# microsoft/BLAS-on-flash

Measured on NVIDIA B200. Metric: gemm_gflops, higher is better.
Workload: dtype f32

## Files before the change

### blas-on-flash_b200/csrc/common.cuh

```cuda
#pragma once

#include <cuda.h>
#include <cuda_runtime.h>

#include <atomic>
#include <cstdarg>
#include <cstdint>
#include <cstdio>
#include <cstring>
#include <mutex>
#include <string>
#include <vector>

#include "bof_b200.h"

namespace bof {

constexpr int kNumSmsFallback = 148;

struct StageSlot {
  void* ptr = nullptr;
  cudaEvent_t ev = nullptr;
  bool in_flight = false;
  char* out_dst = nullptr;
  size_t out_pitch = 0, out_width = 0, out_rows = 0;
};

class CopyPool;
class Drainer;

}

namespace bof { struct CommState; }

struct bof_ctx {
  bof_config cfg{};
  int device = 0;
  int num_sms = bof::kNumSmsFallback;
  size_t l2_bytes = 0;
  cudaStream_t compute = nullptr;
  cudaStream_t h2d = nullptr;
  cudaStream_t d2h = nullptr;
  std::vector<bof::StageSlot> stage_in, stage_out;
  bof::CopyPool* pool = nullptr;
  bof::CopyPool* pool_out = nullptr;
  bof::Drainer* drainer = nullptr;
  std::string err;
  bof_stats stats{};
  std::atomic<int64_t> launches{0};
  void* tmap_encode = nullptr;
  static constexpr int kSlots = 40;
  void* slot_ptr[kSlots] = {};
  size_t slot_bytes[kSlots] = {};
  std::vector<cudaEvent_t> events;
  struct TraceMark { cudaEvent_t ev; const char* what; int idx; };
  std::vector<TraceMark> trace;
  std::vector<cudaEvent_t> trace_pool;
  struct HostMark { double ms; const char* what; long idx; };
  std::vector<HostMark> host_trace;
  std::mutex host_trace_mu;
  double trace_t0 = 0.0;
  cudaEvent_t tk0 = nullptr, tk1 = nullptr;
  bool tk_valid = false;
  uint32_t* sync_ctr = nullptr;
  size_t sync_ctr_count = 0;
  bof::CommState* comm = nullptr;
  cudaStream_t coll = nullptr;
  int sm_reserve = 0;
};

namespace bof {

struct PerDeviceOnce {
  std::atomic<uint64_t> mask{0};
  bool need(int dev) const { return ((mask.load(std::memory_order_acquire) >> (dev & 63)) & 1ull) == 0; }
  void done(int dev) { mask.fetch_or(1ull << (dev & 63), std::memory_order_release); }
};

inline int fail(bof_ctx* ctx, int code, const char* fmt, ...) {
  char buf[512];
  va_list ap;
  va_start(ap, fmt);
  vsnprintf(buf, sizeof(buf), fmt, ap);
  va_end(ap);
  if (ctx) ctx->err = buf;
  if (getenv("BOF_VERBOSE")) fprintf(stderr, "[bof_b200] error %d: %s\n", code, buf);
  return code;
}

#define BOF_CUDA(ctx, expr)                                                                  \
  do {                                                                                       \
    cudaError_t e__ = (expr);                                                                \
    if (e__ != cudaSuccess)                                                                  \
      return bof::fail((ctx), BOF_ECUDA, "%s failed: %s (%s:%d)", #expr,                     \
                       cudaGetErrorString(e__), __FILE__, __LINE__);                         \
  } while (0)

#define BOF_LAUNCH_CHECK(ctx, what)                                                          \
  do {                                                                                       \
    cudaError_t e__ = cudaGetLastError();                                                    \
    if (e__ != cudaSuccess)                                                                  \
      return bof::fail((ctx), BOF_ECUDA, "launch of %s failed: %s (%s:%d)", (what),          \
                       cudaGetErrorString(e__), __FILE__, __LINE__);                         \
    (ctx)->launches.fetch_add(1, std::memory_order_relaxed);                                 \
  } while (0)

#define BOF_REQUIRE(ctx, cond, ...)                                                          \
  do {                                                                                       \
    if (!(cond)) return bof::fail((ctx), BOF_EINVAL, __VA_ARGS__);                           \
  } while (0)

template <typename T>
__host__ __device__ constexpr T ceil_div(T a, T b) {
  return (a + b - 1) / b;
}
template <typename T>
__host__ __device__ constexpr T round_up(T a, T b) {
  return ceil_div(a, b) * b;
}

inline bool aligned16(const void* p) { return (reinterpret_cast<uintptr_t>(p) & 15) == 0; }

int slot_reserve(bof_ctx* ctx, int slot, size_t bytes, void** out);
template <typename T>
int slot_reserve(bof_ctx* ctx, int slot, size_t count, T** out) {
  void* p = nullptr;
  int rc = slot_reserve(ctx, slot, count * sizeof(T), &p);
  *out = static_cast<T*>(p);
  return rc;
}


int launch_spmm_rm(bof_ctx* ctx, cudaStream_t s, int64_t m, int64_t k, float alpha,
                   const float* vals, const int32_t* idx, const int64_t* offs, const float* B,
                   int64_t ldb, float beta, float* C, int64_t ldc, int64_t b_rows = 0);
int launch_spmv(bof_ctx* ctx, cudaStream_t s, char trans, int64_t m, int64_t n, const float* vals,
                const int32_t* idx, const int64_t* offs, const float* x, float* y, int64_t nnz = -1);
size_t spmv_t_workspace_bytes(int64_t n, int64_t nnz);
int launch_spmv_t_sorted(bof_ctx* ctx, cudaStream_t s, int accumulate, int64_t m, int64_t n, int64_t nnz, const float* vals,
                         const int32_t* idx, const int64_t* offs, const float* x, float* y, void* ws, size_t ws_bytes);
constexpr int kSlotSpmvT = 35;
constexpr int kSlotSpmmLong = 36;
int launch_idx_narrow(bof_ctx* ctx, cudaStream_t s, const int64_t* in, int32_t* out, int64_t n);
int launch_idx_widen(bof_ctx* ctx, cudaStream_t s, const int32_t* in, int64_t* out, int64_t n);
int launch_transpose(bof_ctx* ctx, cudaStream_t s, int64_t rows, int64_t cols, const float* in,
                     int64_t ldi, float* out, int64_t ldo);
int launch_add_outer_terms(bof_ctx* ctx, cudaStream_t s, float* C, int64_t rows, int64_t cols, int64_t ldc,
                           const float* rowv, const float* colv, int row_first);
int launch_transpose_axpby(bof_ctx* ctx, cudaStream_t s, int64_t rows, int64_t cols, float alpha,
                           const float* in, int64_t ldi, float beta, float* out, int64_t ldo);

int launch_split_planes(bof_ctx* ctx, cudaStream_t s, int64_t R, int64_t K, const float* src,
                        int64_t s_r, int64_t s_k, float* hi, float* lo, int64_t kp);

struct GemmEpilogue {
  float alpha = 1.f, beta = 0.f;
  float* C = nullptr;
  int64_t ldc = 0;
  const float* row_add = nullptr;
  const float* col_add = nullptr;
  int32_t* argmin_out = nullptr;
  const float* carry = nullptr;
  int64_t ld_carry = 0;
  bool raw_out = false;
};

int launch_gemm_tc(bof_ctx* ctx, cudaStream_t s, int cta_group, int64_t M, int64_t N, int64_t K,
                   int64_t kp, const float* p_hi, const float* p_lo, const float* q_hi,
                   const float* q_lo, const GemmEpilogue& ep, int64_t k_chunk);

int tc_issue_rate(bof_ctx* ctx, cudaStream_t s, int kind, int rounds, double* mma_tflops, double* useful_tflops);

int launch_gemm_ffma(bof_ctx* ctx, cudaStream_t s, int64_t M, int64_t N, int64_t K, float alpha,
                     const float* A, int64_t a_r, int64_t a_k, const float* B, int64_t b_k,
                     int64_t b_c, float beta, float* C, int64_t ldc);

int launch_row_sqnorm(bof_ctx* ctx, cudaStream_t s, int64_t rows, int64_t dim, const float* X,
                      int64_t ldx, float* out);
size_t kmeans_reduce_workspace_bytes(int64_t npoints, int64_t ncenters, int64_t dim);
int launch_kmeans_reduce_ws(bof_ctx* ctx, cudaStream_t s, int64_t npoints, int64_t ncenters,
                            int64_t dim, const float* points, const int32_t* assign, float* sums,
                            float* counts, void* ws, size_t ws_bytes, float* counts_hi = nullptr);
int launch_kmeans_finalize(bof_ctx* ctx, cudaStream_t s, int64_t ncenters, int64_t dim,
                           const float* sums, const float* counts, float* centers, float* c_l2sq,
                           const float* counts_hi = nullptr);

size_t csr2csc_workspace_bytes(int64_t m, int64_t n, int64_t nnz);
int launch_csr2csc(bof_ctx* ctx, cudaStream_t s, int64_t m, int64_t n, int64_t nnz,
                   const int64_t* offs, const int32_t* idx, const float* vals, int64_t* offs_t,
                   int32_t* idx_t, float* vals_t, void* ws, size_t ws_bytes);

}
```

### blas-on-flash_b200/csrc/gemm_tc.cu

```cuda
#include "common.cuh"

#include <cuda_bf16.h>

#ifndef BOF_DEFAULT_HYBRID
#define BOF_DEFAULT_HYBRID 1
#endif

namespace bof {
namespace tc {

constexpr int BLOCK_M = 128;
constexpr int BLOCK_K = 32;
constexpr int UMMA_K = 8;
constexpr int LOAD_N = 128;
constexpr int STAGES = 3;
constexpr int PLANE_BYTES = 128 * BLOCK_K * 4;
constexpr int STAGE_BYTES = 4 * PLANE_BYTES;
constexpr int NUM_THREADS = 384;
constexpr int NUM_EPI_WARPS = 8;
constexpr uint32_t PEER_BIT_MASK = 0xFEFFFFFFu;

enum EpiMode { EPI_GEMM = 0, EPI_ARGMIN = 1 };

struct Params {
  int64_t M, N;
  int32_t num_kb;
  int32_t kb_per_chunk;
  int32_t tiles_m, tiles_n;
  int32_t n_per_item;
  float alpha, beta;
  float* C;
  int64_t ldc;
  const float* row_add;
  const float* col_add;
  int32_t* argmin_out;
  uint32_t* sync_counters;
  int32_t sync_kb;
  const float* carry;
  int64_t ld_carry;
  int32_t raw_out;
};

__device__ __forceinline__ uint32_t smem_u32(const void* p) {
  return static_cast<uint32_t>(__cvta_generic_to_shared(p));
}
__device__ __forceinline__ uint32_t cluster_ctarank() {
  uint32_t r;
  asm volatile("mov.u32 %0, %%cluster_ctarank;" : "=r"(r));
  return r;
}
__device__ __forceinline__ void cluster_sync_all() {
  asm volatile("barrier.cluster.arrive.release.aligned;\n\tbarrier.cluster.wait.acquire.aligned;" ::: "memory");
}
__device__ __forceinline__ void mbar_init(uint64_t* bar, uint32_t count) {
  asm volatile("mbarrier.init.shared::cta.b64 [%0], %1;" ::"r"(smem_u32(bar)), "r"(count));
}
__device__ __forceinline__ void fence_barrier_init() {
  asm volatile("fence.mbarrier_init.release.cluster;" ::: "memory");
}
__device__ __forceinline__ uint64_t globaltimer_ns() {
  uint64_t t;
  asm volatile("mov.u64 %0, %%globaltimer;" : "=l"(t));
  return t;
}
__device__ __forceinline__ void mbar_wait(uint64_t* bar, uint32_t parity) {
  const uint32_t addr = smem_u32(bar);
  uint32_t done = 0;
  uint64_t t0 = 0;
  uint32_t spins = 0;
  while (true) {
    asm volatile(
        "{\n\t.reg .pred p;\n\t"
        "mbarrier.try_wait.parity.shared::cta.b64 p, [%1], %2;\n\t"
        "selp.u32 %0, 1, 0, p;\n\t}"
        : "=r"(done)
        : "r"(addr), "r"(parity)
        : "memory");
    if (done) break;
    if ((++spins & 0xfffu) == 0) {
      const uint64_t now = globaltimer_ns();
      if (t0 == 0) t0 = now;
      else if (now - t0 > 4000000000ull) __trap();
    }
  }
}
__device__ __forceinline__ void mbar_arrive_expect_tx(uint64_t* bar, uint32_t bytes) {
  asm volatile("mbarrier.arrive.expect_tx.shared::cta.b64 _, [%0], %1;" ::"r"(smem_u32(bar)), "r"(bytes)
               : "memory");
}
__device__ __forceinline__ void mbar_arrive_leader(uint64_t* bar) {
  asm volatile("mbarrier.arrive.shared::cluster.b64 _, [%0];" ::"r"(smem_u32(bar) & PEER_BIT_MASK) : "memory");
}

template <int CG>
__device__ __forceinline__ void tma_load_2d(const CUtensorMap* map, uint64_t* full_bar, void* dst,
                                            int32_t c_inner, int32_t c_outer) {
  if constexpr (CG == 2) {
    asm volatile(
        "cp.async.bulk.tensor.2d.cta_group::2.shared::cluster.global.mbarrier::complete_tx::bytes"
        " [%0], [%1, {%3, %4}], [%2];" ::"r"(smem_u32(dst)),
        "l"(reinterpret_cast<uint64_t>(map)), "r"(smem_u32(full_bar) & PEER_BIT_MASK), "r"(c_inner),
        "r"(c_outer)
        : "memory");
  } else {
    asm volatile(
        "cp.async.bulk.tensor.2d.shared::cluster.global.mbarrier::complete_tx::bytes"
        " [%0], [%1, {%3, %4}], [%2];" ::"r"(smem_u32(dst)),
        "l"(reinterpret_cast<uint64_t>(map)), "r"(smem_u32(full_bar)), "r"(c_inner), "r"(c_outer)
        : "memory");
  }
}

template <int CG>
__device__ __forceinline__ void tmem_alloc(uint32_t* dst_smem, uint32_t ncols) {
  if constexpr (CG == 2) {
    asm volatile("tcgen05.alloc.cta_group::2.sync.aligned.shared::cta.b32 [%0], %1;" ::"r"(smem_u32(dst_smem)), "r"(ncols) : "memory");
    asm volatile("tcgen05.relinquish_alloc_permit.cta_group::2.sync.aligned;" ::: "memory");
  } else {
    asm volatile("tcgen05.alloc.cta_group::1.sync.aligned.shared::cta.b32 [%0], %1;" ::"r"(smem_u32(dst_smem)), "r"(ncols) : "memory");
    asm volatile("tcgen05.relinquish_alloc_permit.cta_group::1.sync.aligned;" ::: "memory");
  }
}
template <int CG>
__device__ __forceinline__ void tmem_dealloc(uint32_t taddr, uint32_t ncols) {
  if constexpr (CG == 2)
    asm volatile("tcgen05.dealloc.cta_group::2.sync.aligned.b32 %0, %1;" ::"r"(taddr), "r"(ncols) : "memory");
  else
    asm volatile("tcgen05.dealloc.cta_group::1.sync.aligned.b32 %0, %1;" ::"r"(taddr), "r"(ncols) : "memory");
}
__device__ __forceinline__ void tc_fence_before() {
  asm volatile("tcgen05.fence::before_thread_sync;" ::: "memory");
}
__device__ __forceinline__ void tc_fence_after() {
  asm volatile("tcgen05.fence::after_thread_sync;" ::: "memory");
}

template <int CG>
__device__ __forceinline__ void umma_tf32(uint32_t tmem_d, uint64_t desc_a, uint64_t desc_b,
                                          uint32_t idesc, uint32_t accumulate) {
  if constexpr (CG == 2) {
    asm volatile(
        "{\n\t.reg .pred p;\n\tsetp.ne.b32 p, %4, 0;\n\t"
        "tcgen05.mma.cta_group::2.kind::tf32 [%0], %1, %2, %3, p;\n\t}" ::"r"(tmem_d),
        "l"(desc_a), "l"(desc_b), "r"(idesc), "r"(accumulate)
        : "memory");
  } else {
    asm volatile(
        "{\n\t.reg .pred p;\n\tsetp.ne.b32 p, %4, 0;\n\t"
        "tcgen05.mma.cta_group::1.kind::tf32 [%0], %1, %2, %3, p;\n\t}" ::"r"(tmem_d),
        "l"(desc_a), "l"(desc_b), "r"(idesc), "r"(accumulate)
        : "memory");
  }
}
template <int CG>
__device__ __forceinline__ void umma_bf16(uint32_t tmem_d, uint64_t desc_a, uint64_t desc_b,
                                          uint32_t idesc, uint32_t accumulate) {
  if constexpr (CG == 2) {
    asm volatile(
        "{\n\t.reg .pred p;\n\tsetp.ne.b32 p, %4, 0;\n\t"
        "tcgen05.mma.cta_group::2.kind::f16 [%0], %1, %2, %3, p;\n\t}" ::"r"(tmem_d),
        "l"(desc_a), "l"(desc_b), "r"(idesc), "r"(accumulate)
        : "memory");
  } else {
    asm volatile(
        "{\n\t.reg .pred p;\n\tsetp.ne.b32 p, %4, 0;\n\t"
        "tcgen05.mma.cta_group::1.kind::f16 [%0], %1, %2, %3, p;\n\t}" ::"r"(tmem_d),
        "l"(desc_a), "l"(desc_b), "r"(idesc), "r"(accumulate)
        : "memory");
  }
}
template <int CG>
__device__ __forceinline__ void umma_commit(uint64_t* bar) {
  if constexpr (CG == 2) {
    const uint16_t mask = 0b11;
    asm volatile(
        "tcgen05.commit.cta_group::2.mbarrier::arrive::one.shared::cluster.multicast::cluster.b64 [%0], %1;" ::"r"(
            smem_u32(bar)),
        "h"(mask)
        : "memory");
  } else {
    asm volatile("tcgen05.commit.cta_group::1.mbarrier::arrive::one.shared::cluster.b64 [%0];" ::"r"(smem_u32(bar))
                 : "memory");
  }
}
__device__ __forceinline__ void tmem_ld32(uint32_t taddr, uint32_t (&v)[32]) {
  asm volatile(
      "tcgen05.ld.sync.aligned.32x32b.x32.b32 "
      "{%0, %1, %2, %3, %4, %5, %6, %7, %8, %9, %10, %11, %12, %13, %14, %15, "
      "%16, %17, %18, %19, %20, %21, %22, %23, %24, %25, %26, %27, %28, %29, %30, %31}, [%32];"
      : "=r"(v[0]), "=r"(v[1]), "=r"(v[2]), "=r"(v[3]), "=r"(v[4]), "=r"(v[5]), "=r"(v[6]),
        "=r"(v[7]), "=r"(v[8]), "=r"(v[9]), "=r"(v[10]), "=r"(v[11]), "=r"(v[12]), "=r"(v[13]),
        "=r"(v[14]), "=r"(v[15]), "=r"(v[16]), "=r"(v[17]), "=r"(v[18]), "=r"(v[19]), "=r"(v[20]),
        "=r"(v[21]), "=r"(v[22]), "=r"(v[23]), "=r"(v[24]), "=r"(v[25]), "=r"(v[26]), "=r"(v[27]),
        "=r"(v[28]), "=r"(v[29]), "=r"(v[30]), "=r"(v[31])
      : "r"(taddr)
      : "memory");
}
__device__ __forceinline__ void tmem_ld_wait() {
  asm volatile("tcgen05.wait::ld.sync.aligned;" ::: "memory");
}

__device__ __forceinline__ uint64_t make_smem_desc(uint32_t saddr) {
  uint64_t d = 0;
  d |= (uint64_t)((saddr >> 4) & 0x3FFF);
  d |= (uint64_t)1 << 16;
  d |= (uint64_t)(1024 >> 4) << 32;
  d |= (uint64_t)1 << 46;
  d |= (uint64_t)2 << 61;
  return d;
}
__host__ __device__ constexpr uint32_t make_idesc(int umma_m, int umma_n, uint32_t fmt = 2u) {
  return (1u << 4)
         | (fmt << 7) | (fmt << 10)
         | ((uint32_t)(umma_n >> 3) << 17) | ((uint32_t)(umma_m >> 4) << 24);
}

template <int N>
__device__ __forceinline__ void setmaxnreg_inc() {
  asm volatile("setmaxnreg.inc.sync.aligned.u32 %0;" ::"n"(N));
}
template <int N>
__device__ __forceinline__ void setmaxnreg_dec() {
  asm volatile("setmaxnreg.dec.sync.aligned.u32 %0;" ::"n"(N));
}

struct SmemTail {
  uint64_t full[STAGES];
  uint64_t empty[STAGES];
  uint64_t tmem_full[2];
  uint64_t tmem_empty[2];
  uint32_t tmem_base;
  uint32_t pad;
  float red_val[BLOCK_M];
  int32_t red_idx[BLOCK_M];
};

constexpr size_t SMEM_BYTES = (size_t)STAGES * STAGE_BYTES + sizeof(SmemTail) + 1024;

template <int CG, int EPI, bool CHUNKED, bool HYB, bool FOLD = false>
__global__ void __launch_bounds__(NUM_THREADS, 1)
gemm3xtf32_kernel(const __grid_constant__ CUtensorMap map_p_hi, const __grid_constant__ CUtensorMap map_p_lo,
                  const __grid_constant__ CUtensorMap map_q_hi, const __grid_constant__ CUtensorMap map_q_lo,
                  const Params prm) {
  constexpr int BLOCK_N = (CG == 2) ? 256 : 128;
  constexpr int TILE_M = BLOCK_M * CG;
  constexpr int EPI_COLS = BLOCK_N / 2;
  constexpr uint32_t TMEM_COLS = 2 * BLOCK_N;
  constexpr uint32_t IDESC = make_idesc(BLOCK_M * CG, BLOCK_N, 2u);
  constexpr uint32_t IDESC_BF16 = make_idesc(BLOCK_M * CG, BLOCK_N, 1u);
  static_assert(!FOLD || (EPI == EPI_GEMM && CHUNKED), "the fold carry exists for the chunked GEMM epilogue only");

  extern __shared__ uint8_t smem_raw[];
  uint8_t* smem = reinterpret_cast<uint8_t*>((reinterpret_cast<uintptr_t>(smem_raw) + 1023) & ~(uintptr_t)1023);
  SmemTail* tail = reinterpret_cast<SmemTail*>(smem + (size_t)STAGES * STAGE_BYTES);

  const int warp = threadIdx.x >> 5;
  const int lane = threadIdx.x & 31;
  const uint32_t cta_rank = (CG == 2) ? cluster_ctarank() : 0u;
  const bool is_leader = cta_rank == 0;
  const int cluster_id = blockIdx.x / CG;
  const int num_clusters = gridDim.x / CG;

  if (warp == 1 && lane == 0) {
    for (int s = 0; s < STAGES; ++s) {
      mbar_init(&tail->full[s], CG);
      mbar_init(&tail->empty[s], 1);
    }
    for (int b = 0; b < 2; ++b) {
      mbar_init(&tail->tmem_full[b], 1);
      mbar_init(&tail->tmem_empty[b], NUM_EPI_WARPS * CG);
    }
    fence_barrier_init();
  }
  if (warp == 2) tmem_alloc<CG>(&tail->tmem_base, TMEM_COLS);
  tc_fence_before();
  if constexpr (CG == 2) cluster_sync_all(); else __syncthreads();
  tc_fence_after();
  const uint32_t tmem_base = tail->tmem_base;

  const int num_items = (EPI == EPI_ARGMIN) ? prm.tiles_m : prm.tiles_m * prm.tiles_n;
  const int num_chunks = (prm.num_kb + prm.kb_per_chunk - 1) / prm.kb_per_chunk;

  auto decode_item = [&](int item, int& tm, int& tn0) {
    if (EPI == EPI_ARGMIN) { tm = item; tn0 = 0; return; }
    constexpr int GROUP = 8;
    const int per_group = GROUP * prm.tiles_n;
    const int g = item / per_group;
    const int first_m = g * GROUP;
    const int gsz = min(GROUP, prm.tiles_m - first_m);
    const int r = item - g * per_group;
    tm = first_m + r % gsz;
    tn0 = r / gsz;
  };

  if (warp < 4) {
    if constexpr (CHUNKED) setmaxnreg_dec<40>();
    if (warp == 0) {
      int stage = 0;
      uint32_t phase = 0;
      for (int item = cluster_id; item < num_items; item += num_clusters) {
        int tm, tn0;
        decode_item(item, tm, tn0);
        const int32_t row_p = tm * TILE_M + (int)cta_rank * BLOCK_M;
        for (int nt = 0; nt < prm.n_per_item; ++nt) {
          const int32_t row_q = (tn0 + nt) * BLOCK_N + (int)cta_rank * LOAD_N;
          for (int kb = 0; kb < prm.num_kb; ++kb) {
            mbar_wait(&tail->empty[stage], phase ^ 1);
            if (EPI == EPI_GEMM && prm.sync_kb > 0 && is_leader && lane == 0 && kb % prm.sync_kb == 0) {
              const int wave = (item - cluster_id) / num_clusters;
              const int syncs_per_tile = (prm.num_kb + prm.sync_kb - 1) / prm.sync_kb;
              const uint32_t expected = (uint32_t)min(num_clusters, num_items - wave * num_clusters);
              uint32_t* ctr = prm.sync_counters + (size_t)wave * syncs_per_tile + kb / prm.sync_kb;
              asm volatile("red.release.gpu.global.add.u32 [%0], 1;" ::"l"(ctr) : "memory");
              uint32_t seen = 0;
              const uint64_t t0 = globaltimer_ns();
              for (uint32_t spins = 0;; ++spins) {
                asm volatile("ld.acquire.gpu.global.u32 %0, [%1];" : "=r"(seen) : "l"(ctr) : "memory");
                if (seen >= expected) break;
                __nanosleep(100);
                if ((spins & 0x3fu) == 0x3fu && globaltimer_ns() - t0 > 500000ull) break;
              }
            }
            if (lane == 0) {
              uint8_t* st = smem + (size_t)stage * STAGE_BYTES;
              if (is_leader) mbar_arrive_expect_tx(&tail->full[stage], STAGE_BYTES * CG);
              else mbar_arrive_leader(&tail->full[stage]);
              const int32_t kc = kb * BLOCK_K;
              tma_load_2d<CG>(&map_p_hi, &tail->full[stage], st, kc, row_p);
              tma_load_2d<CG>(&map_p_lo, &tail->full[stage], st + PLANE_BYTES, kc, row_p);
              tma_load_2d<CG>(&map_q_hi, &tail->full[stage], st + 2 * PLANE_BYTES, kc, row_q);
              tma_load_2d<CG>(&map_q_lo, &tail->full[stage], st + 3 * PLANE_BYTES, kc, row_q);
            }
            __syncwarp();
            if (++stage == STAGES) { stage = 0; phase ^= 1; }
          }
        }
      }
    } else if (warp == 1 && is_leader) {
      int stage = 0;
      uint32_t phase = 0;
      uint32_t acc_iter = 0;
      for (int item = cluster_id; item < num_items; item += num_clusters) {
        for (int nt = 0; nt < prm.n_per_item; ++nt) {
          for (int c = 0; c < num_chunks; ++c, ++acc_iter) {
            const uint32_t buf = acc_iter & 1u;
            mbar_wait(&tail->tmem_empty[buf], ((acc_iter >> 1) & 1u) ^ 1u);
            tc_fence_after();
            const uint32_t tmem_d = tmem_base + buf * BLOCK_N;
            const int kb_end = min(prm.num_kb, (c + 1) * prm.kb_per_chunk);
            for (int kb = c * prm.kb_per_chunk; kb < kb_end; ++kb) {
              mbar_wait(&tail->full[stage], phase);
              tc_fence_after();
              if (lane == 0) {
                const uint32_t st = smem_u32(smem + (size_t)stage * STAGE_BYTES);
                const uint64_t d_p_hi = make_smem_desc(st);
                const uint64_t d_p_lo = make_smem_desc(st + PLANE_BYTES);
                const uint64_t d_q_hi = make_smem_desc(st + 2 * PLANE_BYTES);
                const uint64_t d_q_lo = make_smem_desc(st + 3 * PLANE_BYTES);
                const uint32_t fresh = (kb == c * prm.kb_per_chunk) ? 0u : 1u;
                if constexpr (HYB) {
#pragma unroll
                  for (int kk = 0; kk < 2; ++kk) {
                    const uint64_t adv = (uint64_t)(kk * 2);
                    umma_bf16<CG>(tmem_d, d_p_lo + 4 + adv, d_q_lo + adv, IDESC_BF16, kk == 0 ? fresh : 1u);
                    umma_bf16<CG>(tmem_d, d_p_lo + adv, d_q_lo + 4 + adv, IDESC_BF16, 1u);
                  }
#pragma unroll
                  for (int kk = 0; kk < BLOCK_K / UMMA_K; ++kk) {
                    const uint64_t adv = (uint64_t)((kk * UMMA_K * 4) >> 4);
                    umma_tf32<CG>(tmem_d, d_p_hi + adv, d_q_hi + adv, IDESC, 1u);
                  }
                } else {
#pragma unroll
                  for (int kk = 0; kk < BLOCK_K / UMMA_K; ++kk) {
                    const uint64_t adv = (uint64_t)((kk * UMMA_K * 4) >> 4);
                    umma_tf32<CG>(tmem_d, d_p_lo + adv, d_q_hi + adv, IDESC, kk == 0 ? fresh : 1u);
                    umma_tf32<CG>(tmem_d, d_p_hi + adv, d_q_lo + adv, IDESC, 1u);
                    umma_tf32<CG>(tmem_d, d_p_hi + adv, d_q_hi + adv, IDESC, 1u);
                  }
                }
                umma_commit<CG>(&tail->empty[stage]);
                if (kb == kb_end - 1) umma_commit<CG>(&tail->tmem_full[buf]);
              }
              __syncwarp();
              if (++stage == STAGES) { stage = 0; phase ^= 1; }
            }
          }
        }
      }
    }
  } else {
    if constexpr (CHUNKED) setmaxnreg_inc<232>();
    const int e = warp - 4;
    const int quarter = e & 3;
    const int half = e >> 2;
    const int row_in_tile = (int)cta_rank * BLOCK_M + quarter * 32 + lane;
    const uint32_t lane_addr = (uint32_t)(quarter * 32) << 16;
    uint32_t acc_iter = 0;

    for (int item = cluster_id; item < num_items; item += num_clusters) {
      int tm, tn0;
      decode_item(item, tm, tn0);
      const int64_t row = (int64_t)tm * TILE_M + row_in_tile;
      float best = 3.402823466e+38f;
      int32_t best_idx = 0x7fffffff;
      float radd = 0.f;
      if (EPI == EPI_ARGMIN && row < prm.M) radd = __ldg(prm.row_add + row);

      for (int nt = 0; nt < prm.n_per_item; ++nt) {
        const int64_t col0 = (int64_t)(tn0 + nt) * BLOCK_N + half * EPI_COLS;
        float acc[CHUNKED ? EPI_COLS : 1];
        for (int c = 0; c < num_chunks; ++c, ++acc_iter) {
          const uint32_t buf = acc_iter & 1u;
          mbar_wait(&tail->tmem_full[buf], (acc_iter >> 1) & 1u);
          tc_fence_after();
          const uint32_t taddr = tmem_base + lane_addr + buf * BLOCK_N + half * EPI_COLS;
#pragma unroll
          for (int g = 0; g < EPI_COLS / 32; ++g) {
            uint32_t v[32];
            tmem_ld32(taddr + g * 32, v);
            tmem_ld_wait();
            if constexpr (CHUNKED) {
              if (FOLD && c == 0 && prm.carry != nullptr && row < prm.M) {
                const float* krow = prm.carry + row * prm.ld_carry + col0 + g * 32;
#pragma unroll
                for (int j = 0; j < 32; ++j)
                  acc[g * 32 + j] = (col0 + g * 32 + j < prm.N) ? krow[j] + __uint_as_float(v[j]) : __uint_as_float(v[j]);
              } else if (c == 0) {
#pragma unroll
                for (int j = 0; j < 32; ++j) acc[g * 32 + j] = __uint_as_float(v[j]);
              } else {
#pragma unroll
                for (int j = 0; j < 32; ++j) acc[g * 32 + j] += __uint_as_float(v[j]);
              }
            } else {
              if constexpr (EPI == EPI_GEMM) {
                if (row < prm.M) {
                  float* crow = prm.C + row * prm.ldc + col0 + g * 32;
#pragma unroll
                  for (int j = 0; j < 32; ++j) {
                    if (col0 + g * 32 + j < prm.N) {
                      float r = prm.alpha * __uint_as_float(v[j]);
                      if (prm.beta != 0.f) r = fmaf(prm.beta, crow[j], r);
                      crow[j] = r;
                    }
                  }
                }
              } else {
#pragma unroll
                for (int j = 0; j < 32; ++j) {
                  const int64_t cj = col0 + g * 32 + j;
                  if (cj < prm.N) {
                    float d = __fadd_rn(__fadd_rn(-2.f * __uint_as_float(v[j]), __ldg(prm.col_add + cj)), radd);
                    d = fabsf(d);
                    if (d < best) { best = d; best_idx = (int32_t)cj; }
                  }
                }
              }
            }
          }
          tc_fence_before();
          __syncwarp();
          if (lane == 0) mbar_arrive_leader(&tail->tmem_empty[buf]);
        }
        if constexpr (CHUNKED) {
          if constexpr (EPI == EPI_GEMM) {
            if (row < prm.M) {
              float* crow = prm.C + row * prm.ldc + col0;
#pragma unroll
              for (int j = 0; j < EPI_COLS; ++j) {
                if (FOLD && prm.raw_out) {
                  if (col0 + j < prm.N) crow[j] = acc[j];
                } else if (col0 + j < prm.N) {
                  float r = prm.alpha * acc[j];
                  if (prm.beta != 0.f) r = fmaf(prm.beta, crow[j], r);
                  crow[j] = r;
                }
              }
            }
          } else {
#pragma unroll
            for (int j = 0; j < EPI_COLS; ++j) {
              const int64_t cj = col0 + j;
              if (cj < prm.N) {
                float d = __fadd_rn(__fadd_rn(-2.f * acc[j], __ldg(prm.col_add + cj)), radd);
                d = fabsf(d);
                if (d < best) { best = d; best_idx = (int32_t)cj; }
              }
            }
          }
        }
      }

      if constexpr (EPI == EPI_ARGMIN) {
        const int r_local = quarter * 32 + lane;
        if (half == 1) {
          tail->red_val[r_local] = best;
          tail->red_idx[r_local] = best_idx;
        }
        asm volatile("bar.sync 1, 256;" ::: "memory");
        if (half == 0) {
          const float ov = tail->red_val[r_local];
          const int32_t oi = tail->red_idx[r_local];
          if (ov < best || (ov == best && oi < best_idx)) { best = ov; best_idx = oi; }
          if ((uint32_t)best_idx >= (uint32_t)prm.N) best_idx = 0;
          if (row < prm.M) prm.argmin_out[row] = best_idx;
        }
        asm volatile("bar.sync 1, 256;" ::: "memory");
      }
    }
  }

  tc_fence_before();
  if constexpr (CG == 2) cluster_sync_all(); else __syncthreads();
  if (warp == 2) tmem_dealloc<CG>(tmem_base, TMEM_COLS);
}


__global__ void __launch_bounds__(128, 1)
tc_issue_rate_kernel(int kind, int rounds) {
  constexpr int CG = 2;
  constexpr int BLOCK_N = 256;
  constexpr uint32_t IDESC = make_idesc(BLOCK_M * CG, BLOCK_N, 2u);
  constexpr uint32_t IDESC_BF16 = make_idesc(BLOCK_M * CG, BLOCK_N, 1u);
  extern __shared__ uint8_t smem_raw[];
  uint8_t* smem = reinterpret_cast<uint8_t*>((reinterpret_cast<uintptr_t>(smem_raw) + 1023) & ~(uintptr_t)1023);
  __shared__ uint64_t done_bar;
  __shared__ uint32_t tmem_base_s;
  const int warp = threadIdx.x >> 5, lane = threadIdx.x & 31;
  const bool is_leader = cluster_ctarank() == 0;
  uint32_t* w = reinterpret_cast<uint32_t*>(smem);
  for (int i = threadIdx.x; i < STAGE_BYTES / 4; i += blockDim.x) w[i] = 0x3f800000u + ((i * 2654435761u) & 0x007f0000u);
  if (threadIdx.x == 0) { mbar_init(&done_bar, 1); fence_barrier_init(); }
  if (warp == 2) tmem_alloc<CG>(&tmem_base_s, 2 * BLOCK_N);
  asm volatile("fence.proxy.async.shared::cta;" ::: "memory");
  tc_fence_before();
  cluster_sync_all();
  tc_fence_after();
  const uint32_t tmem_d = tmem_base_s;
  if (warp == 1 && is_leader) {
    if (lane == 0) {
      const uint32_t st = smem_u32(smem);
      const uint64_t d_p_hi = make_smem_desc(st), d_p_lo = make_smem_desc(st + PLANE_BYTES);
      const uint64_t d_q_hi = make_smem_desc(st + 2 * PLANE_BYTES), d_q_lo = make_smem_desc(st + 3 * PLANE_BYTES);
      for (int r = 0; r < rounds; ++r) {
        if (kind != 0) {
#pragma unroll
          for (int kk = 0; kk < 2; ++kk) {
            const uint64_t adv = (uint64_t)(kk * 2);
            umma_bf16<CG>(tmem_d, d_p_lo + 4 + adv, d_q_lo + adv, IDESC_BF16, (r | kk) == 0 ? 0u : 1u);
            umma_bf16<CG>(tmem_d, d_p_lo + adv, d_q_lo + 4 + adv, IDESC_BF16, 1u);
          }
        }
        if (kind != 1) {
#pragma unroll
          for (int kk = 0; kk < BLOCK_K / UMMA_K; ++kk) {
            const uint64_t adv = (uint64_t)((kk * UMMA_K * 4) >> 4);
            umma_tf32<CG>(tmem_d, d_p_hi + adv, d_q_hi + adv, IDESC, (kind == 0 && (r | kk) == 0) ? 0u : 1u);
          }
        }
      }
      umma_commit<CG>(&done_bar);
    }
    __syncwarp();
  }
  if (warp == 0) mbar_wait(&done_bar, 0);
  tc_fence_before();
  cluster_sync_all();
  if (warp == 2) tmem_dealloc<CG>(tmem_d, 2 * BLOCK_N);
}

}

namespace {

__device__ __forceinline__ float rna_tf32(float x) {
  uint32_t u;
  asm("cvt.rna.tf32.f32 %0, %1;" : "=r"(u) : "f"(x));
  return __uint_as_float(u);
}

struct SplitElem {
  float hi, lo;
  uint16_t bh, bl;
};
__device__ __forceinline__ SplitElem split_elem(float x) {
  SplitElem s;
  const uint32_t ax = __float_as_uint(x) & 0x7fffffffu;
  if (ax >= 0x7f800000u) {
    s.hi = x; s.lo = 0.f; s.bh = 0; s.bl = 0;
    return s;
  }
  s.hi = ax >= 0x7f7ff000u ? __uint_as_float(__float_as_uint(x) & ~0x1fffu) : rna_tf32(x);
  const float e = x - s.hi;
  s.lo = rna_tf32(e);
  const uint32_t ah = __float_as_uint(s.hi) & 0x7fffffffu;
  s.bh = ah >= 0x7f7f8000u ? (uint16_t)(__float_as_uint(s.hi) >> 16) : __bfloat16_as_ushort(__float2bfloat16_rn(s.hi));
  s.bl = __bfloat16_as_ushort(__float2bfloat16_rn(e));
  return s;
}
__device__ __forceinline__ uint8_t* combo_ptr(float* plane, int64_t r, int64_t kp, int64_t kk, bool lo_half) {
  return reinterpret_cast<uint8_t*>(plane + r * kp) + (kk >> 5) * 128 + (lo_half ? 64 : 0) + (kk & 31) * 2;
}

__global__ void __launch_bounds__(256)
split_planes_kmajor_kernel(int64_t R, int64_t K, const float* __restrict__ src, int64_t s_r,
                           float* __restrict__ hi, float* __restrict__ lo, int64_t kp, bool vec, bool combo) {
  const int64_t quads_per_row = kp / 4;
  const int64_t total = R * quads_per_row;
  const int64_t stride = (int64_t)gridDim.x * blockDim.x;
  for (int64_t q = (int64_t)blockIdx.x * blockDim.x + threadIdx.x; q < total; q += stride) {
    const int64_t r = q / quads_per_row, k0 = (q - r * quads_per_row) * 4;
    float x[4] = {0.f, 0.f, 0.f, 0.f};
    const float* p = src + r * s_r + k0;
    if (vec && k0 + 4 <= K) {
      const float4 t = __ldcs(reinterpret_cast<const float4*>(p));
      x[0] = t.x; x[1] = t.y; x[2] = t.z; x[3] = t.w;
    } else {
#pragma unroll
      for (int u = 0; u < 4; ++u)
        if (k0 + u < K) x[u] = p[u];
    }
    const SplitElem s0 = split_elem(x[0]), s1 = split_elem(x[1]), s2 = split_elem(x[2]), s3 = split_elem(x[3]);
    *reinterpret_cast<float4*>(hi + r * kp + k0) = make_float4(s0.hi, s1.hi, s2.hi, s3.hi);
    if (!combo) {
      *reinterpret_cast<float4*>(lo + r * kp + k0) = make_float4(s0.lo, s1.lo, s2.lo, s3.lo);
    } else {
      uint2 ph, pl;
      ph.x = s0.bh | ((uint32_t)s1.bh << 16);
      ph.y = s2.bh | ((uint32_t)s3.bh << 16);
      pl.x = s0.bl | ((uint32_t)s1.bl << 16);
      pl.y = s2.bl | ((uint32_t)s3.bl << 16);
      *reinterpret_cast<uint2*>(combo_ptr(lo, r, kp, k0, false)) = ph;
      *reinterpret_cast<uint2*>(combo_ptr(lo, r, kp, k0, true)) = pl;
    }
  }
}

__global__ void __launch_bounds__(256)
split_planes_transpose_kernel(int64_t R, int64_t K, const float* __restrict__ src, int64_t s_k,
                              float* __restrict__ hi, float* __restrict__ lo, int64_t kp,
                              unsigned tiles_k, bool combo) {
  __shared__ float tile[32][33];
  const int tx = threadIdx.x & 31, ty = threadIdx.x >> 5;
  const int64_t r0 = (int64_t)(blockIdx.x / tiles_k) * 32, k0 = (int64_t)(blockIdx.x % tiles_k) * 32;
#pragma unroll
  for (int i = ty; i < 32; i += 8) {
    const int64_t kk = k0 + i, r = r0 + tx;
    tile[i][tx] = (kk < K && r < R) ? src[kk * s_k + r] : 0.f;
  }
  __syncthreads();
#pragma unroll
  for (int i = ty; i < 32; i += 8) {
    const int64_t r = r0 + i, kk = k0 + tx;
    if (r < R && kk < kp) {
      const SplitElem sp = split_elem(tile[tx][i]);
      hi[r * kp + kk] = sp.hi;
      if (!combo) {
        lo[r * kp + kk] = sp.lo;
      } else {
        *reinterpret_cast<uint16_t*>(combo_ptr(lo, r, kp, kk, false)) = sp.bh;
        *reinterpret_cast<uint16_t*>(combo_ptr(lo, r, kp, kk, true)) = sp.bl;
      }
    }
  }
}

__global__ void __launch_bounds__(256)
gemm_ffma_kernel(int64_t M, int64_t N, int64_t K, float alpha, const float* __restrict__ A,
                 int64_t a_r, int64_t a_k, const float* __restrict__ B, int64_t b_k, int64_t b_c,
                 float beta, float* __restrict__ C, int64_t ldc) {
  constexpr int BM = 64, BN = 64, BK = 16;
  __shared__ float As[BK][BM + 4];
  __shared__ float Bs[BK][BN + 4];
  const int tid = threadIdx.x;
  const int tx = tid & 15, ty = tid >> 4;
  const int64_t m0 = (int64_t)blockIdx.y * BM, n0 = (int64_t)blockIdx.x * BN;
  float acc[4][4] = {};
  for (int64_t k0 = 0; k0 < K; k0 += BK) {
    for (int i = tid; i < BM * BK; i += 256) {
      int mm, kk;
      if (a_k == 1) { kk = i % BK; mm = i / BK; } else { mm = i % BM; kk = i / BM; }
      const int64_t gm = m0 + mm, gk = k0 + kk;
      As[kk][mm] = (gm < M && gk < K) ? A[gm * a_r + gk * a_k] : 0.f;
    }
    for (int i = tid; i < BN * BK; i += 256) {
      int nn, kk;
      if (b_k == 1) { kk = i % BK; nn = i / BK; } else { nn = i % BN; kk = i / BN; }
      const int64_t gn = n0 + nn, gk = k0 + kk;
      Bs[kk][nn] = (gn < N && gk < K) ? B[gk * b_k + gn * b_c] : 0.f;
    }
    __syncthreads();
#pragma unroll
    for (int kk = 0; kk < BK; ++kk) {
      float a[4], b[4];
#pragma unroll
      for (int u = 0; u < 4; ++u) { a[u] = As[kk][ty * 4 + u]; b[u] = Bs[kk][tx * 4 + u]; }
#pragma unroll
      for (int u = 0; u < 4; ++u)
#pragma unroll
        for (int v = 0; v < 4; ++v) acc[u][v] = fmaf(a[u], b[v], acc[u][v]);
    }
    __syncthreads();
  }
#pragma unroll
  for (int u = 0; u < 4; ++u) {
    const int64_t gm = m0 + ty * 4 + u;
    if (gm >= M) continue;
#pragma unroll
    for (int v = 0; v < 4; ++v) {
      const int64_t gn = n0 + tx * 4 + v;
      if (gn >= N) continue;
      float r = alpha * acc[u][v];
      if (beta != 0.f) r = fmaf(beta, C[gm * ldc + gn], r);
      C[gm * ldc + gn] = r;
    }
  }
}

bool hybrid_split(const bof_ctx* ctx) { return ctx->cfg.gemm_split == 2 || (ctx->cfg.gemm_split == 0 && BOF_DEFAULT_HYBRID); }

typedef CUresult (*EncodeTiledFn)(CUtensorMap*, CUtensorMapDataType, cuuint32_t, void*, const cuuint64_t*,
                                  const cuuint64_t*, const cuuint32_t*, const cuuint32_t*,
                                  CUtensorMapInterleave, CUtensorMapSwizzle, CUtensorMapL2promotion,
                                  CUtensorMapFloatOOBfill);

int make_plane_map(bof_ctx* ctx, CUtensorMap* map, const float* plane, int64_t rows, int64_t kp) {
  BOF_REQUIRE(ctx, ctx->tmap_encode != nullptr, "cuTensorMapEncodeTiled unavailable");
  const cuuint64_t dims[2] = {(cuuint64_t)kp, (cuuint64_t)rows};
  const cuuint64_t strides[1] = {(cuuint64_t)kp * sizeof(float)};
  const cuuint32_t box[2] = {(cuuint32_t)tc::BLOCK_K, 128u};
  const cuuint32_t estr[2] = {1u, 1u};
  CUresult r = reinterpret_cast<EncodeTiledFn>(ctx->tmap_encode)(
      map, CU_TENSOR_MAP_DATA_TYPE_FLOAT32, 2, const_cast<float*>(plane), dims, strides, box, estr,
      CU_TENSOR_MAP_INTERLEAVE_NONE, CU_TENSOR_MAP_SWIZZLE_128B, CU_TENSOR_MAP_L2_PROMOTION_L2_256B,
      CU_TENSOR_MAP_FLOAT_OOB_FILL_NONE);
  if (r != CUDA_SUCCESS) return fail(ctx, BOF_ECUDA, "cuTensorMapEncodeTiled failed with CUresult %d", (int)r);
  return BOF_OK;
}

template <int CG, int EPI, bool CHUNKED, bool HYB, bool FOLD = false>
int launch_variant(bof_ctx* ctx, cudaStream_t s, const CUtensorMap* maps, const tc::Params& prm, int num_items) {
  auto kern = tc::gemm3xtf32_kernel<CG, EPI, CHUNKED, HYB, FOLD>;
  static PerDeviceOnce attr_set;
  if (attr_set.need(ctx->device)) {
    BOF_CUDA(ctx, cudaFuncSetAttribute(kern, cudaFuncAttributeMaxDynamicSharedMemorySize, (int)tc::SMEM_BYTES));
    attr_set.done(ctx->device);
  }
  const int max_clusters = std::max(1, (ctx->num_sms - ctx->sm_reserve) / CG);
  const int clusters = std::max(1, std::min(num_items, max_clusters));
  cudaLaunchConfig_t cfg{};
  cfg.gridDim = dim3((unsigned)(clusters * CG));
  cfg.blockDim = dim3(tc::NUM_THREADS);
  cfg.dynamicSmemBytes = tc::SMEM_BYTES;
  cfg.stream = s;
  cudaLaunchAttribute attr[1];
  attr[0].id = cudaLaunchAttributeClusterDimension;
  attr[0].val.clusterDim.x = CG;
  attr[0].val.clusterDim.y = 1;
  attr[0].val.clusterDim.z = 1;
  cfg.attrs = attr;
  cfg.numAttrs = 1;
  if (!ctx->tk0) {
    BOF_CUDA(ctx, cudaEventCreate(&ctx->tk0));
    BOF_CUDA(ctx, cudaEventCreate(&ctx->tk1));
  }
  BOF_CUDA(ctx, cudaEventRecord(ctx->tk0, s));
  BOF_CUDA(ctx, cudaLaunchKernelEx(&cfg, kern, maps[0], maps[1], maps[2], maps[3], prm));
  BOF_LAUNCH_CHECK(ctx, "gemm3xtf32_kernel");
  BOF_CUDA(ctx, cudaEventRecord(ctx->tk1, s));
  ctx->tk_valid = true;
  return BOF_OK;
}

}

int launch_split_planes(bof_ctx* ctx, cudaStream_t s, int64_t R, int64_t K, const float* src,
                        int64_t s_r, int64_t s_k, float* hi, float* lo, int64_t kp) {
  BOF_REQUIRE(ctx, kp % 32 == 0 && kp >= K, "split: bad padded k");
  if (R == 0) return BOF_OK;
  if (s_k == 1) {
    const bool vec = (s_r % 4 == 0) && aligned16(src);
    const int64_t total = R * (kp / 4);
    const unsigned grid = (unsigned)std::min<int64_t>(ceil_div<int64_t>(total, 256), (int64_t)ctx->num_sms * 32);
    split_planes_kmajor_kernel<<<grid, 256, 0, s>>>(R, K, src, s_r, hi, lo, kp, vec, hybrid_split(ctx));
    BOF_LAUNCH_CHECK(ctx, "split_planes_kmajor_kernel");
  } else {
    BOF_REQUIRE(ctx, s_r == 1, "split: one of the operand strides must be 1");
    const int64_t tiles_k = kp / 32, tiles_r = ceil_div<int64_t>(R, 32);
    BOF_REQUIRE(ctx, tiles_k * tiles_r < (1ll << 31), "split: operand too large for one launch");
    split_planes_transpose_kernel<<<(unsigned)(tiles_k * tiles_r), 256, 0, s>>>(R, K, src, s_k, hi, lo, kp,
                                                                               (unsigned)tiles_k, hybrid_split(ctx));
    BOF_LAUNCH_CHECK(ctx, "split_planes_transpose_kernel");
  }
  return BOF_OK;
}

int launch_gemm_tc(bof_ctx* ctx, cudaStream_t s, int cta_group, int64_t M, int64_t N, int64_t K,
                   int64_t kp, const float* p_hi, const float* p_lo, const float* q_hi,
                   const float* q_lo, const GemmEpilogue& ep, int64_t k_chunk) {
  (void)K;
  if (M == 0 || N == 0) return BOF_OK;
  BOF_REQUIRE(ctx, cta_group == 1 || cta_group == 2, "gemm_tc: cta_group must be 1 or 2");
  BOF_REQUIRE(ctx, kp % 32 == 0 && kp > 0, "gemm_tc: padded k must be a positive multiple of 32");
  BOF_REQUIRE(ctx, M < (1ll << 31) && N < (1ll << 31) && kp < (1ll << 31), "gemm_tc: extent exceeds int32");
  CUtensorMap maps[4];
  int rc;
  if ((rc = make_plane_map(ctx, &maps[0], p_hi, M, kp))) return rc;
  if ((rc = make_plane_map(ctx, &maps[1], p_lo, M, kp))) return rc;
  if ((rc = make_plane_map(ctx, &maps[2], q_hi, N, kp))) return rc;
  if ((rc = make_plane_map(ctx, &maps[3], q_lo, N, kp))) return rc;

  const int block_n = cta_group == 2 ? 256 : 128;
  const int tile_m = 128 * cta_group;
  tc::Params prm{};
  prm.M = M;
  prm.N = N;
  prm.num_kb = (int32_t)(kp / 32);
  int64_t kbc = (k_chunk <= 0) ? prm.num_kb : std::max<int64_t>(1, k_chunk / 32);
  if (kbc > prm.num_kb) kbc = prm.num_kb;
  prm.kb_per_chunk = (int32_t)kbc;
  prm.tiles_m = (int32_t)ceil_div<int64_t>(M, tile_m);
  prm.tiles_n = (int32_t)ceil_div<int64_t>(N, block_n);
  const bool argmin = ep.C == nullptr;
  prm.n_per_item = argmin ? prm.tiles_n : 1;
  prm.alpha = ep.alpha;
  prm.beta = ep.beta;
  prm.C = ep.C;
  prm.ldc = ep.ldc;
  prm.row_add = ep.row_add;
  prm.col_add = ep.col_add;
  prm.argmin_out = ep.argmin_out;
  prm.carry = ep.carry;
  prm.ld_carry = ep.ld_carry;
  prm.raw_out = ep.raw_out ? 1 : 0;
  const bool fold = ep.carry != nullptr || ep.raw_out;
  if (argmin)
    BOF_REQUIRE(ctx, ep.row_add && ep.col_add && ep.argmin_out, "gemm_tc: argmin epilogue needs norms and an output");
  BOF_REQUIRE(ctx, !(argmin && fold), "gemm_tc: the fold carry needs the GEMM epilogue");
  const bool chunked = prm.kb_per_chunk < prm.num_kb;
  const int num_items = argmin ? prm.tiles_m : prm.tiles_m * prm.tiles_n;
  const int clusters = std::max(1, std::min(num_items, std::max(1, (ctx->num_sms - ctx->sm_reserve) / cta_group)));
  prm.sync_kb = 0;
  prm.sync_counters = nullptr;
  if (!argmin && ctx->cfg.gemm_wave_sync >= 0 && prm.num_kb >= 256 && num_items > clusters) {
    prm.sync_kb = ctx->cfg.gemm_wave_sync > 0 ? ctx->cfg.gemm_wave_sync : 64;
    const size_t waves = (size_t)ceil_div(num_items, clusters);
    const size_t n_ctr = waves * (size_t)ceil_div(prm.num_kb, prm.sync_kb);
    if (ctx->sync_ctr_count < n_ctr) {
      size_t n_alloc = 1u << 16;
      while (n_alloc < n_ctr) n_alloc <<= 1;
      if (ctx->sync_ctr) BOF_CUDA(ctx, cudaFree(ctx->sync_ctr));
      ctx->sync_ctr = nullptr;
      ctx->sync_ctr_count = 0;
      BOF_CUDA(ctx, cudaMalloc(&ctx->sync_ctr, n_alloc * sizeof(uint32_t)));
      ctx->sync_ctr_count = n_alloc;
    }
    BOF_CUDA(ctx, cudaMemsetAsync(ctx->sync_ctr, 0, n_ctr * sizeof(uint32_t), s));
    prm.sync_counters = ctx->sync_ctr;
  }

  const bool hyb = hybrid_split(ctx);
  if (fold) {
    if (cta_group == 2) {
      if (hyb) return launch_variant<2, tc::EPI_GEMM, true, true, true>(ctx, s, maps, prm, num_items);
      return launch_variant<2, tc::EPI_GEMM, true, false, true>(ctx, s, maps, prm, num_items);
    }
    if (hyb) return launch_variant<1, tc::EPI_GEMM, true, true, true>(ctx, s, maps, prm, num_items);
    return launch_variant<1, tc::EPI_GEMM, true, false, true>(ctx, s, maps, prm, num_items);
  }
#define BOF_TC(CG, EPI, CH)                                                            \
  do {                                                                                 \
    if (hyb) return launch_variant<CG, EPI, CH, true>(ctx, s, maps, prm, num_items);   \
    return launch_variant<CG, EPI, CH, false>(ctx, s, maps, prm, num_items);           \
  } while (0)
  if (cta_group == 2) {
    if (argmin) { if (chunked) BOF_TC(2, tc::EPI_ARGMIN, true); else BOF_TC(2, tc::EPI_ARGMIN, false); }
    if (chunked) BOF_TC(2, tc::EPI_GEMM, true); else BOF_TC(2, tc::EPI_GEMM, false);
  } else {
    if (argmin) { if (chunked) BOF_TC(1, tc::EPI_ARGMIN, true); else BOF_TC(1, tc::EPI_ARGMIN, false); }
    if (chunked) BOF_TC(1, tc::EPI_GEMM, true); else BOF_TC(1, tc::EPI_GEMM, false);
  }
#undef BOF_TC
}

int launch_gemm_ffma(bof_ctx* ctx, cudaStream_t s, int64_t M, int64_t N, int64_t K, float alpha,
                     const float* A, int64_t a_r, int64_t a_k, const float* B, int64_t b_k,
                     int64_t b_c, float beta, float* C, int64_t ldc) {
  if (M == 0 || N == 0) return BOF_OK;
  dim3 grid((unsigned)ceil_div<int64_t>(N, 64), (unsigned)ceil_div<int64_t>(M, 64));
  BOF_REQUIRE(ctx, grid.y <= 65535u, "gemm_ffma: too many row tiles (use the tensor-core path)");
  gemm_ffma_kernel<<<grid, 256, 0, s>>>(M, N, K, alpha, A, a_r, a_k, B, b_k, b_c, beta, C, ldc);
  BOF_LAUNCH_CHECK(ctx, "gemm_ffma_kernel");
  return BOF_OK;
}


int tc_issue_rate(bof_ctx* ctx, cudaStream_t s, int kind, int rounds, double* mma_tflops, double* useful_tflops) {
  BOF_REQUIRE(ctx, kind >= 0 && kind <= 2 && rounds > 0, "tc_issue_rate: bad kind / rounds");
  static PerDeviceOnce attr_set;
  const size_t smem = (size_t)tc::STAGE_BYTES + 2048;
  if (attr_set.need(ctx->device)) {
    BOF_CUDA(ctx, cudaFuncSetAttribute(tc::tc_issue_rate_kernel, cudaFuncAttributeMaxDynamicSharedMemorySize, (int)smem));
    attr_set.done(ctx->device);
  }
  const int clusters = ctx->num_sms / 2;
  cudaLaunchConfig_t cfg{};
  cfg.gridDim = dim3((unsigned)(clusters * 2));
  cfg.blockDim = dim3(128);
  cfg.dynamicSmemBytes = smem;
  cfg.stream = s;
  cudaLaunchAttribute attr[1];
  attr[0].id = cudaLaunchAttributeClusterDimension;
  attr[0].val.clusterDim.x = 2; attr[0].val.clusterDim.y = 1; attr[0].val.clusterDim.z = 1;
  cfg.attrs = attr; cfg.numAttrs = 1;
  cudaEvent_t e0, e1;
  BOF_CUDA(ctx, cudaEventCreate(&e0));
  BOF_CUDA(ctx, cudaEventCreate(&e1));
  BOF_CUDA(ctx, cudaLaunchKernelEx(&cfg, tc::tc_issue_rate_kernel, kind, 64));
  BOF_CUDA(ctx, cudaEventRecord(e0, s));
  BOF_CUDA(ctx, cudaLaunchKernelEx(&cfg, tc::tc_issue_rate_kernel, kind, rounds));
  BOF_LAUNCH_CHECK(ctx, "tc_issue_rate_kernel");
  BOF_CUDA(ctx, cudaEventRecord(e1, s));
  BOF_CUDA(ctx, cudaStreamSynchronize(s));
  float ms = 0.f;
  BOF_CUDA(ctx, cudaEventElapsedTime(&ms, e0, e1));
  cudaEventDestroy(e0); cudaEventDestroy(e1);
  const double per_round_useful = 2.0 * 256 * 256 * 32;
  const double mma_per_round = per_round_useful * (kind == 2 ? 3.0 : (kind == 1 ? 2.0 : 1.0));
  if (mma_tflops) *mma_tflops = mma_per_round * rounds * clusters / (ms * 1e-3) / 1e12;
  if (useful_tflops) *useful_tflops = per_round_useful * rounds * clusters / (ms * 1e-3) / 1e12;
  return BOF_OK;
}

}
```

### blas-on-flash_b200/csrc/host_internal.cuh

```cuda
#pragma once

#include "common.cuh"

#include <algorithm>
#include <cstdint>
#include <cstdlib>
#include <string>
#include <vector>

#define BOF_TRY(expr)          \
  do {                         \
    int rc__ = (expr);         \
    if (rc__ != BOF_OK) return rc__; \
  } while (0)

namespace bof {

constexpr int kGemmRing = 5;

inline bool is_nt(char c) { return c == 'N' || c == 'T'; }
inline bool is_rc(char c) { return c == 'R' || c == 'C'; }
inline cudaStream_t as_stream(void* s) { return reinterpret_cast<cudaStream_t>(s); }

enum Slot {
  S_DENSE = 0,
  S_DENSE_T,
  S_BLK0 = 2,
  S_OFFS = 2, S_IDX64 = 4, S_IDX32 = 6, S_VALS = 8, S_CBLK = 10, S_CBLK_T = 12,
  S_WS = 18,
  S_OUT0 = 19, S_OUT1, S_OUT2, S_MISC,
  S_PRAW = 24, S_PPLANES = 30, S_GCBLK = 32,
};

double now_ms();
cudaEvent_t get_event(bof_ctx* ctx, size_t i);
bool trace_on();
void trace_mark(bof_ctx* ctx, cudaStream_t s, const char* what, int idx);
void trace_host(bof_ctx* ctx, const char* what, long idx);
void trace_dump(bof_ctx* ctx, const char* title);
bool host_is_pinned(const void* p);
int copy2d(bof_ctx* ctx, void* dst, size_t dpitch, const void* src, size_t spitch, size_t width, size_t height,
           cudaMemcpyKind kind, cudaStream_t s);
int copy1d(bof_ctx* ctx, void* dst, const void* src, size_t bytes, cudaMemcpyKind kind, cudaStream_t s);
int d2h_transfer(bof_ctx* ctx, void* dst, size_t dpitch, const void* src, size_t spitch, size_t width, size_t height,
                 cudaStream_t s, cudaEvent_t wait_ev, cudaEvent_t record_ev, uint64_t* ticket);
void d2h_fence(bof_ctx* ctx, uint64_t ticket);
void stats_begin(bof_ctx* ctx);
void stats_end(bof_ctx* ctx);
int drain_wait(bof_ctx* ctx);
int sync_all(bof_ctx* ctx);
void quiesce(bof_ctx* ctx);
void staging_destroy(bof_ctx* ctx);

struct CallGuard {
  bof_ctx* ctx;
  bool ok = false;
  explicit CallGuard(bof_ctx* c) : ctx(c) {}
  ~CallGuard() { if (!ok && ctx) quiesce(ctx); }
  int done() { ok = true; return BOF_OK; }
};

struct Canon {
  int64_t Mo, No, K;
  const float* psrc; int64_t p_sr, p_sk;
  const float* qsrc; int64_t q_sr, q_sk;
  int64_t ldc;
};
int canon_gemm(bof_ctx* ctx, char ord, char ta, char tb, int64_t m, int64_t n, int64_t k,
               const float* A, int64_t lda, const float* B, int64_t ldb, int64_t ldc, Canon* out);
int64_t padded_k(int64_t k);
size_t plane_bytes(int64_t rows, int64_t kp);
int pick_gemm_path(const bof_ctx* ctx, int64_t Mo, int64_t No, int64_t K);
int64_t k_chunk_of(const bof_ctx* ctx);
int gemm_canon_device(bof_ctx* ctx, cudaStream_t s, const Canon& c, float alpha, float beta, float* C,
                      void* ws, size_t ws_bytes);

int comm_world(const bof_ctx* ctx);
int comm_rank(const bof_ctx* ctx);
int comm_broadcast_f32(bof_ctx* ctx, float* buf, size_t count, int root);
int comm_allreduce_sum_f32(bof_ctx* ctx, float* buf, size_t count, cudaStream_t s);
void comm_destroy(bof_ctx* ctx);
int comm_exchange_begin(bof_ctx* ctx, size_t bytes, float** xbuf_out);
int comm_push(bof_ctx* ctx, size_t offset, size_t count, int item, cudaEvent_t ready);
int comm_wait_item(bof_ctx* ctx, cudaStream_t s, int item);
void comm_sync_pushes(bof_ctx* ctx);

std::vector<int64_t> partition_rows(const int64_t* ia, int64_t m, int64_t max_nnz);

}
```

Before: 343,800.

## Add fp16-high split with per-chunk exponent scaling for emulated FP32 GEMM

Adds a third split mode, now the default. The high plane is stored as per-chunk-scaled fp16 instead of tf32, and the two low-order terms stay bf16. The high-by-high product runs as an f16 UMMA over half-width smem tiles with 64B swizzle, and the stage ring grows from 3 to 4 stages in the same shared memory. The epilogue undoes the per-row and per-column power-of-two scales using exponents stored in the plane padding. This is meant to cut tensor-core issue cost and smem/TMA bytes for the dominant term, at the price of extra epilogue work, a heavier split pre-pass, and accuracy risk from fp16 range and scaling.

```diff
diff --git a/blas-on-flash_b200/csrc/common.cuh b/blas-on-flash_b200/csrc/common.cuh
--- a/blas-on-flash_b200/csrc/common.cuh
+++ b/blas-on-flash_b200/csrc/common.cuh
@@ -150,6 +150,8 @@
 int launch_transpose_axpby(bof_ctx* ctx, cudaStream_t s, int64_t rows, int64_t cols, float alpha,
                            const float* in, int64_t ldi, float beta, float* out, int64_t ldo);
 
+int64_t k_chunk_of(const bof_ctx* ctx);
+
 int launch_split_planes(bof_ctx* ctx, cudaStream_t s, int64_t R, int64_t K, const float* src,
                         int64_t s_r, int64_t s_k, float* hi, float* lo, int64_t kp);
 
diff --git a/blas-on-flash_b200/csrc/gemm_tc.cu b/blas-on-flash_b200/csrc/gemm_tc.cu
--- a/blas-on-flash_b200/csrc/gemm_tc.cu
+++ b/blas-on-flash_b200/csrc/gemm_tc.cu
@@ -1,9 +1,10 @@
 #include "common.cuh"
 
 #include <cuda_bf16.h>
-
-#ifndef BOF_DEFAULT_HYBRID
-#define BOF_DEFAULT_HYBRID 1
+#include <cuda_fp16.h>
+
+#ifndef BOF_DEFAULT_SPLIT
+#define BOF_DEFAULT_SPLIT 3
 #endif
 
 namespace bof {
@@ -16,6 +17,9 @@
 constexpr int STAGES = 3;
 constexpr int PLANE_BYTES = 128 * BLOCK_K * 4;
 constexpr int STAGE_BYTES = 4 * PLANE_BYTES;
+constexpr int STAGES_F16 = 4;
+constexpr int HI16_BYTES = 128 * BLOCK_K * 2;
+constexpr int STAGE_BYTES_F16 = 2 * HI16_BYTES + 2 * PLANE_BYTES;
 constexpr int NUM_THREADS = 384;
 constexpr int NUM_EPI_WARPS = 8;
 constexpr uint32_t PEER_BIT_MASK = 0xFEFFFFFFu;
@@ -39,6 +43,9 @@
   const float* carry;
   int64_t ld_carry;
   int32_t raw_out;
+  const int16_t* p_exp;
+  const int16_t* q_exp;
+  int64_t exp_ld;
 };
 
 __device__ __forceinline__ uint32_t smem_u32(const void* p) {
@@ -196,6 +203,16 @@
       : "r"(taddr)
       : "memory");
 }
+__device__ __forceinline__ void tmem_ld16(uint32_t taddr, uint32_t (&v)[16]) {
+  asm volatile(
+      "tcgen05.ld.sync.aligned.32x32b.x16.b32 "
+      "{%0, %1, %2, %3, %4, %5, %6, %7, %8, %9, %10, %11, %12, %13, %14, %15}, [%16];"
+      : "=r"(v[0]), "=r"(v[1]), "=r"(v[2]), "=r"(v[3]), "=r"(v[4]), "=r"(v[5]), "=r"(v[6]), "=r"(v[7]),
+        "=r"(v[8]), "=r"(v[9]), "=r"(v[10]), "=r"(v[11]), "=r"(v[12]), "=r"(v[13]), "=r"(v[14]), "=r"(v[15])
+      : "r"(taddr)
+      : "memory");
+}
+__device__ __forceinline__ float pow2i(int e) { return __int_as_float((127 + e) << 23); }
 __device__ __forceinline__ void tmem_ld_wait() {
   asm volatile("tcgen05.wait::ld.sync.aligned;" ::: "memory");
 }
@@ -209,6 +226,15 @@
   d |= (uint64_t)2 << 61;
   return d;
 }
+__device__ __forceinline__ uint64_t make_smem_desc_sw64(uint32_t saddr) {
+  uint64_t d = 0;
+  d |= (uint64_t)((saddr >> 4) & 0x3FFF);
+  d |= (uint64_t)1 << 16;
+  d |= (uint64_t)(512 >> 4) << 32;
+  d |= (uint64_t)1 << 46;
+  d |= (uint64_t)4 << 61;
+  return d;
+}
 __host__ __device__ constexpr uint32_t make_idesc(int umma_m, int umma_n, uint32_t fmt = 2u) {
   return (1u << 4)
          | (fmt << 7) | (fmt << 10)
@@ -225,8 +251,8 @@
 }
 
 struct SmemTail {
-  uint64_t full[STAGES];
-  uint64_t empty[STAGES];
+  uint64_t full[STAGES_F16];
+  uint64_t empty[STAGES_F16];
   uint64_t tmem_full[2];
   uint64_t tmem_empty[2];
   uint32_t tmem_base;
@@ -235,9 +261,10 @@
   int32_t red_idx[BLOCK_M];
 };
 
+static_assert(STAGES_F16 * STAGE_BYTES_F16 == STAGES * STAGE_BYTES, "both stage rings fill the same smem");
 constexpr size_t SMEM_BYTES = (size_t)STAGES * STAGE_BYTES + sizeof(SmemTail) + 1024;
 
-template <int CG, int EPI, bool CHUNKED, bool HYB, bool FOLD = false>
+template <int CG, int EPI, bool CHUNKED, int SPLIT, bool FOLD = false>
 __global__ void __launch_bounds__(NUM_THREADS, 1)
 gemm3xtf32_kernel(const __grid_constant__ CUtensorMap map_p_hi, const __grid_constant__ CUtensorMap map_p_lo,
                   const __grid_constant__ CUtensorMap map_q_hi, const __grid_constant__ CUtensorMap map_q_lo,
@@ -248,6 +275,12 @@
   constexpr uint32_t TMEM_COLS = 2 * BLOCK_N;
   constexpr uint32_t IDESC = make_idesc(BLOCK_M * CG, BLOCK_N, 2u);
   constexpr uint32_t IDESC_BF16 = make_idesc(BLOCK_M * CG, BLOCK_N, 1u);
+  constexpr uint32_t IDESC_F16 = make_idesc(BLOCK_M * CG, BLOCK_N, 0u);
+  constexpr bool HYB = SPLIT >= 2;
+  constexpr bool F16 = SPLIT == 3;
+  constexpr int NST = F16 ? STAGES_F16 : STAGES;
+  constexpr int HI_BYTES = F16 ? HI16_BYTES : PLANE_BYTES;
+  constexpr int ST_BYTES = F16 ? STAGE_BYTES_F16 : STAGE_BYTES;
   static_assert(!FOLD || (EPI == EPI_GEMM && CHUNKED), "the fold carry exists for the chunked GEMM epilogue only");
 
   extern __shared__ uint8_t smem_raw[];
@@ -262,7 +295,7 @@
   const int num_clusters = gridDim.x / CG;
 
   if (warp == 1 && lane == 0) {
-    for (int s = 0; s < STAGES; ++s) {
+    for (int s = 0; s < NST; ++s) {
       mbar_init(&tail->full[s], CG);
       mbar_init(&tail->empty[s], 1);
     }
@@ -322,17 +355,17 @@
               }
             }
             if (lane == 0) {
-              uint8_t* st = smem + (size_t)stage * STAGE_BYTES;
-              if (is_leader) mbar_arrive_expect_tx(&tail->full[stage], STAGE_BYTES * CG);
+              uint8_t* st = smem + (size_t)stage * ST_BYTES;
+              if (is_leader) mbar_arrive_expect_tx(&tail->full[stage], ST_BYTES * CG);
               else mbar_arrive_leader(&tail->full[stage]);
               const int32_t kc = kb * BLOCK_K;
               tma_load_2d<CG>(&map_p_hi, &tail->full[stage], st, kc, row_p);
-              tma_load_2d<CG>(&map_p_lo, &tail->full[stage], st + PLANE_BYTES, kc, row_p);
-              tma_load_2d<CG>(&map_q_hi, &tail->full[stage], st + 2 * PLANE_BYTES, kc, row_q);
-              tma_load_2d<CG>(&map_q_lo, &tail->full[stage], st + 3 * PLANE_BYTES, kc, row_q);
+              tma_load_2d<CG>(&map_p_lo, &tail->full[stage], st + HI_BYTES, kc, row_p);
+              tma_load_2d<CG>(&map_q_hi, &tail->full[stage], st + HI_BYTES + PLANE_BYTES, kc, row_q);
+              tma_load_2d<CG>(&map_q_lo, &tail->full[stage], st + 2 * HI_BYTES + PLANE_BYTES, kc, row_q);
             }
             __syncwarp();
-            if (++stage == STAGES) { stage = 0; phase ^= 1; }
+            if (++stage == NST) { stage = 0; phase ^= 1; }
           }
         }
       }
@@ -352,11 +385,12 @@
               mbar_wait(&tail->full[stage], phase);
               tc_fence_after();
               if (lane == 0) {
-                const uint32_t st = smem_u32(smem + (size_t)stage * STAGE_BYTES);
-                const uint64_t d_p_hi = make_smem_desc(st);
-                const uint64_t d_p_lo = make_smem_desc(st + PLANE_BYTES);
-                const uint64_t d_q_hi = make_smem_desc(st + 2 * PLANE_BYTES);
-                const uint64_t d_q_lo = make_smem_desc(st + 3 * PLANE_BYTES);
+                const uint32_t st = smem_u32(smem + (size_t)stage * ST_BYTES);
+                const uint64_t d_p_hi = F16 ? make_smem_desc_sw64(st) : make_smem_desc(st);
+                const uint64_t d_p_lo = make_smem_desc(st + HI_BYTES);
+                const uint64_t d_q_hi = F16 ? make_smem_desc_sw64(st + HI_BYTES + PLANE_BYTES)
+                                            : make_smem_desc(st + HI_BYTES + PLANE_BYTES);
+                const uint64_t d_q_lo = make_smem_desc(st + 2 * HI_BYTES + PLANE_BYTES);
                 const uint32_t fresh = (kb == c * prm.kb_per_chunk) ? 0u : 1u;
                 if constexpr (HYB) {
 #pragma unroll
@@ -365,10 +399,18 @@
                     umma_bf16<CG>(tmem_d, d_p_lo + 4 + adv, d_q_lo + adv, IDESC_BF16, kk == 0 ? fresh : 1u);
                     umma_bf16<CG>(tmem_d, d_p_lo + adv, d_q_lo + 4 + adv, IDESC_BF16, 1u);
                   }
-#pragma unroll
-                  for (int kk = 0; kk < BLOCK_K / UMMA_K; ++kk) {
-                    const uint64_t adv = (uint64_t)((kk * UMMA_K * 4) >> 4);
-                    umma_tf32<CG>(tmem_d, d_p_hi + adv, d_q_hi + adv, IDESC, 1u);
+                  if constexpr (F16) {
+#pragma unroll
+                    for (int kk = 0; kk < 2; ++kk) {
+                      const uint64_t adv = (uint64_t)(kk * 2);
+                      umma_bf16<CG>(tmem_d, d_p_hi + adv, d_q_hi + adv, IDESC_F16, 1u);
+                    }
+                  } else {
+#pragma unroll
+                    for (int kk = 0; kk < BLOCK_K / UMMA_K; ++kk) {
+                      const uint64_t adv = (uint64_t)((kk * UMMA_K * 4) >> 4);
+                      umma_tf32<CG>(tmem_d, d_p_hi + adv, d_q_hi + adv, IDESC, 1u);
+                    }
                   }
                 } else {
 #pragma unroll
@@ -383,7 +425,7 @@
                 if (kb == kb_end - 1) umma_commit<CG>(&tail->tmem_full[buf]);
               }
               __syncwarp();
-              if (++stage == STAGES) { stage = 0; phase ^= 1; }
+              if (++stage == NST) { stage = 0; phase ^= 1; }
             }
           }
         }
@@ -412,34 +454,56 @@
         float acc[CHUNKED ? EPI_COLS : 1];
         for (int c = 0; c < num_chunks; ++c, ++acc_iter) {
           const uint32_t buf = acc_iter & 1u;
+          float rf1 = 1.f, rf2 = 1.f;
+          if constexpr (F16) {
+            const int s_row = row < prm.M ? prm.p_exp[row * prm.exp_ld + c] : 0;
+            rf1 = pow2i(-(s_row >> 1));
+            rf2 = pow2i((s_row >> 1) - s_row);
+          }
           mbar_wait(&tail->tmem_full[buf], (acc_iter >> 1) & 1u);
           tc_fence_after();
+          constexpr int LW = F16 ? 16 : 32;
           const uint32_t taddr = tmem_base + lane_addr + buf * BLOCK_N + half * EPI_COLS;
 #pragma unroll
-          for (int g = 0; g < EPI_COLS / 32; ++g) {
-            uint32_t v[32];
-            tmem_ld32(taddr + g * 32, v);
+          for (int g = 0; g < EPI_COLS / LW; ++g) {
+            float cf1 = 1.f, cf2 = 1.f;
+            if constexpr (F16) {
+              const int64_t cj = col0 + g * LW + (lane & (LW - 1));
+              const int t = cj < prm.N ? prm.q_exp[cj * prm.exp_ld + c] : 0;
+              cf1 = pow2i(-(t >> 1));
+              cf2 = pow2i((t >> 1) - t);
+            }
+            uint32_t v[LW];
+            if constexpr (F16) tmem_ld16(taddr + g * LW, v); else tmem_ld32(taddr + g * LW, v);
             tmem_ld_wait();
+            if constexpr (F16) {
+#pragma unroll
+              for (int j = 0; j < LW; ++j) {
+                const float f1 = rf1 * __shfl_sync(0xffffffffu, cf1, j);
+                const float f2 = rf2 * __shfl_sync(0xffffffffu, cf2, j);
+                v[j] = __float_as_uint((__uint_as_float(v[j]) * f1) * f2);
+              }
+            }
             if constexpr (CHUNKED) {
               if (FOLD && c == 0 && prm.carry != nullptr && row < prm.M) {
-                const float* krow = prm.carry + row * prm.ld_carry + col0 + g * 32;
-#pragma unroll
-                for (int j = 0; j < 32; ++j)
-                  acc[g * 32 + j] = (col0 + g * 32 + j < prm.N) ? krow[j] + __uint_as_float(v[j]) : __uint_as_float(v[j]);
+                const float* krow = prm.carry + row * prm.ld_carry + col0 + g * LW;
+#pragma unroll
+                for (int j = 0; j < LW; ++j)
+                  acc[g * LW + j] = (col0 + g * LW + j < prm.N) ? krow[j] + __uint_as_float(v[j]) : __uint_as_float(v[j]);
               } else if (c == 0) {
 #pragma unroll
-                for (int j = 0; j < 32; ++j) acc[g * 32 + j] = __uint_as_float(v[j]);
+                for (int j = 0; j < LW; ++j) acc[g * LW + j] = __uint_as_float(v[j]);
               } else {
 #pragma unroll
-                for (int j = 0; j < 32; ++j) acc[g * 32 + j] += __uint_as_float(v[j]);
+                for (int j = 0; j < LW; ++j) acc[g * LW + j] += __uint_as_float(v[j]);
               }
             } else {
               if constexpr (EPI == EPI_GEMM) {
                 if (row < prm.M) {
-                  float* crow = prm.C + row * prm.ldc + col0 + g * 32;
-#pragma unroll
-                  for (int j = 0; j < 32; ++j) {
-                    if (col0 + g * 32 + j < prm.N) {
+                  float* crow = prm.C + row * prm.ldc + col0 + g * LW;
+#pragma unroll
+                  for (int j = 0; j < LW; ++j) {
+                    if (col0 + g * LW + j < prm.N) {
                       float r = prm.alpha * __uint_as_float(v[j]);
                       if (prm.beta != 0.f) r = fmaf(prm.beta, crow[j], r);
                       crow[j] = r;
@@ -448,8 +512,8 @@
                 }
               } else {
 #pragma unroll
-                for (int j = 0; j < 32; ++j) {
-                  const int64_t cj = col0 + g * 32 + j;
+                for (int j = 0; j < LW; ++j) {
+                  const int64_t cj = col0 + g * LW + j;
                   if (cj < prm.N) {
                     float d = __fadd_rn(__fadd_rn(-2.f * __uint_as_float(v[j]), __ldg(prm.col_add + cj)), radd);
                     d = fabsf(d);
@@ -523,6 +587,7 @@
   constexpr int BLOCK_N = 256;
   constexpr uint32_t IDESC = make_idesc(BLOCK_M * CG, BLOCK_N, 2u);
   constexpr uint32_t IDESC_BF16 = make_idesc(BLOCK_M * CG, BLOCK_N, 1u);
+  constexpr uint32_t IDESC_F16 = make_idesc(BLOCK_M * CG, BLOCK_N, 0u);
   extern __shared__ uint8_t smem_raw[];
   uint8_t* smem = reinterpret_cast<uint8_t*>((reinterpret_cast<uintptr_t>(smem_raw) + 1023) & ~(uintptr_t)1023);
   __shared__ uint64_t done_bar;
@@ -531,6 +596,15 @@
   const bool is_leader = cluster_ctarank() == 0;
   uint32_t* w = reinterpret_cast<uint32_t*>(smem);
   for (int i = threadIdx.x; i < STAGE_BYTES / 4; i += blockDim.x) w[i] = 0x3f800000u + ((i * 2654435761u) & 0x007f0000u);
+  if (kind == 3) {
+    __syncthreads();
+    uint16_t* h = reinterpret_cast<uint16_t*>(smem);
+    for (int i = threadIdx.x; i < PLANE_BYTES / 4; i += blockDim.x) {
+      const uint16_t v = (uint16_t)(0x3c00u + (((uint32_t)i * 2654435761u >> 8) & 0x03f8u));
+      h[i] = v;
+      h[i + PLANE_BYTES] = v;
+    }
+  }
   if (threadIdx.x == 0) { mbar_init(&done_bar, 1); fence_barrier_init(); }
   if (warp == 2) tmem_alloc<CG>(&tmem_base_s, 2 * BLOCK_N);
   asm volatile("fence.proxy.async.shared::cta;" ::: "memory");
@@ -543,6 +617,7 @@
       const uint32_t st = smem_u32(smem);
       const uint64_t d_p_hi = make_smem_desc(st), d_p_lo = make_smem_desc(st + PLANE_BYTES);
       const uint64_t d_q_hi = make_smem_desc(st + 2 * PLANE_BYTES), d_q_lo = make_smem_desc(st + 3 * PLANE_BYTES);
+      const uint64_t d_p_h16 = make_smem_desc_sw64(st), d_q_h16 = make_smem_desc_sw64(st + 2 * PLANE_BYTES);
       for (int r = 0; r < rounds; ++r) {
         if (kind != 0) {
 #pragma unroll
@@ -552,11 +627,17 @@
             umma_bf16<CG>(tmem_d, d_p_lo + adv, d_q_lo + 4 + adv, IDESC_BF16, 1u);
           }
         }
-        if (kind != 1) {
+        if (kind == 0 || kind == 2) {
 #pragma unroll
           for (int kk = 0; kk < BLOCK_K / UMMA_K; ++kk) {
             const uint64_t adv = (uint64_t)((kk * UMMA_K * 4) >> 4);
             umma_tf32<CG>(tmem_d, d_p_hi + adv, d_q_hi + adv, IDESC, (kind == 0 && (r | kk) == 0) ? 0u : 1u);
+          }
+        } else if (kind == 3) {
+#pragma unroll
+          for (int kk = 0; kk < 2; ++kk) {
+            const uint64_t adv = (uint64_t)(kk * 2);
+            umma_bf16<CG>(tmem_d, d_p_h16 + adv, d_q_h16 + adv, IDESC_F16, 1u);
           }
         }
       }
@@ -601,6 +682,105 @@
 }
 __device__ __forceinline__ uint8_t* combo_ptr(float* plane, int64_t r, int64_t kp, int64_t kk, bool lo_half) {
   return reinterpret_cast<uint8_t*>(plane + r * kp) + (kk >> 5) * 128 + (lo_half ? 64 : 0) + (kk & 31) * 2;
+}
+
+__device__ __forceinline__ int chunk_scale_exp(uint32_t amax) {
+  if (amax == 0) return 0;
+  const int e = (int)(amax >> 23) - 127;
+  return min(112, max(-113, 14 - e));
+}
+__device__ __forceinline__ uint32_t finite_abs_bits(float x) {
+  const uint32_t ax = __float_as_uint(x) & 0x7fffffffu;
+  return ax < 0x7f800000u ? ax : 0u;
+}
+struct Split3 {
+  uint16_t h, bh, bl;
+};
+__device__ __forceinline__ Split3 split3_elem(float x, float scale) {
+  Split3 t;
+  if ((__float_as_uint(x) & 0x7fffffffu) >= 0x7f800000u) {
+    t.h = __half_as_ushort(__float2half_rn(x)); t.bh = 0; t.bl = 0;
+    return t;
+  }
+  const float xs = x * scale;
+  const __half h = __float2half_rn(rna_tf32(xs));
+  const float hi = __half2float(h);
+  t.h = __half_as_ushort(h);
+  t.bh = __bfloat16_as_ushort(__float2bfloat16_rn(hi));
+  t.bl = __bfloat16_as_ushort(__float2bfloat16_rn(xs - hi));
+  return t;
+}
+__device__ __forceinline__ uint16_t* hi16_ptr(float* plane, int64_t r, int64_t kp) {
+  return reinterpret_cast<uint16_t*>(plane + r * kp);
+}
+
+__global__ void __launch_bounds__(256)
+split3_kmajor_kernel(int64_t R, int64_t K, const float* __restrict__ src, int64_t s_r, float* __restrict__ hi,
+                     float* __restrict__ lo, int64_t kp, int64_t chunk, int64_t n_chunks) {
+  const int lane = threadIdx.x & 31;
+  const int64_t total = R * n_chunks;
+  const int64_t wstride = (int64_t)gridDim.x * (blockDim.x >> 5);
+  for (int64_t w = ((int64_t)blockIdx.x * blockDim.x + threadIdx.x) >> 5; w < total; w += wstride) {
+    const int64_t r = w / n_chunks, c = w - r * n_chunks;
+    const int64_t k_beg = c * chunk, k_end = min(kp, k_beg + chunk);
+    const float* row = src + r * s_r;
+    uint32_t amax = 0;
+    for (int64_t k = k_beg + lane; k < min(k_end, K); k += 32) amax = max(amax, finite_abs_bits(row[k]));
+#pragma unroll
+    for (int o = 16; o > 0; o >>= 1) amax = max(amax, __shfl_xor_sync(0xffffffffu, amax, o));
+    const int sc = chunk_scale_exp(amax);
+    const float scale = __int_as_float((127 + sc) << 23);
+    uint16_t* h16 = hi16_ptr(hi, r, kp);
+    for (int64_t k = k_beg + lane; k < k_end; k += 32) {
+      const Split3 t = split3_elem(k < K ? row[k] : 0.f, scale);
+      h16[k] = t.h;
+      *reinterpret_cast<uint16_t*>(combo_ptr(lo, r, kp, k, false)) = t.bh;
+      *reinterpret_cast<uint16_t*>(combo_ptr(lo, r, kp, k, true)) = t.bl;
+    }
+    if (lane == 0) reinterpret_cast<int16_t*>(h16 + kp)[c] = (int16_t)sc;
+  }
+}
+
+__global__ void __launch_bounds__(256)
+split3_transpose_kernel(int64_t R, int64_t K, const float* __restrict__ src, int64_t s_k, float* __restrict__ hi,
+                        float* __restrict__ lo, int64_t kp, int64_t chunk, int64_t n_chunks) {
+  __shared__ float tile[32][33];
+  __shared__ uint32_t red[8][32];
+  __shared__ float scale_s[32];
+  const int tx = threadIdx.x & 31, ty = threadIdx.x >> 5;
+  const int64_t r0 = (int64_t)(blockIdx.x / n_chunks) * 32, c = blockIdx.x % n_chunks;
+  const int64_t k_beg = c * chunk, k_end = min(kp, k_beg + chunk);
+  uint32_t amax = 0;
+  if (r0 + tx < R)
+    for (int64_t k = k_beg + ty; k < min(k_end, K); k += 8) amax = max(amax, finite_abs_bits(src[k * s_k + r0 + tx]));
+  red[ty][tx] = amax;
+  __syncthreads();
+  if (ty == 0) {
+#pragma unroll
+    for (int i = 1; i < 8; ++i) amax = max(amax, red[i][tx]);
+    const int sc = chunk_scale_exp(amax);
+    scale_s[tx] = __int_as_float((127 + sc) << 23);
+    if (r0 + tx < R) reinterpret_cast<int16_t*>(hi16_ptr(hi, r0 + tx, kp) + kp)[c] = (int16_t)sc;
+  }
+  for (int64_t k0 = k_beg; k0 < k_end; k0 += 32) {
+    __syncthreads();
+#pragma unroll
+    for (int i = ty; i < 32; i += 8) {
+      const int64_t kk = k0 + i, r = r0 + tx;
+      tile[i][tx] = (kk < K && r < R) ? src[kk * s_k + r] : 0.f;
+    }
+    __syncthreads();
+#pragma unroll
+    for (int i = ty; i < 32; i += 8) {
+      const int64_t r = r0 + i, kk = k0 + tx;
+      if (r < R) {
+        const Split3 t = split3_elem(tile[tx][i], scale_s[i]);
+        hi16_ptr(hi, r, kp)[kk] = t.h;
+        *reinterpret_cast<uint16_t*>(combo_ptr(lo, r, kp, kk, false)) = t.bh;
+        *reinterpret_cast<uint16_t*>(combo_ptr(lo, r, kp, kk, true)) = t.bl;
+      }
+    }
+  }
 }
 
 __global__ void __launch_bounds__(256)
@@ -718,7 +898,15 @@
   }
 }
 
-bool hybrid_split(const bof_ctx* ctx) { return ctx->cfg.gemm_split == 2 || (ctx->cfg.gemm_split == 0 && BOF_DEFAULT_HYBRID); }
+int split_mode(const bof_ctx* ctx) {
+  const int m = ctx->cfg.gemm_split;
+  return (m >= 1 && m <= 3) ? m : BOF_DEFAULT_SPLIT;
+}
+int64_t chunk_kb(int64_t kp, int64_t k_chunk) {
+  const int64_t num_kb = kp / 32;
+  const int64_t kbc = (k_chunk <= 0) ? num_kb : std::max<int64_t>(1, k_chunk / 32);
+  return std::min(kbc, num_kb);
+}
 
 typedef CUresult (*EncodeTiledFn)(CUtensorMap*, CUtensorMapDataType, cuuint32_t, void*, const cuuint64_t*,
                                   const cuuint64_t*, const cuuint32_t*, const cuuint32_t*,
@@ -738,10 +926,23 @@
   if (r != CUDA_SUCCESS) return fail(ctx, BOF_ECUDA, "cuTensorMapEncodeTiled failed with CUresult %d", (int)r);
   return BOF_OK;
 }
-
-template <int CG, int EPI, bool CHUNKED, bool HYB, bool FOLD = false>
+int make_hi16_map(bof_ctx* ctx, CUtensorMap* map, const float* plane, int64_t rows, int64_t kp) {
+  BOF_REQUIRE(ctx, ctx->tmap_encode != nullptr, "cuTensorMapEncodeTiled unavailable");
+  const cuuint64_t dims[2] = {(cuuint64_t)kp, (cuuint64_t)rows};
+  const cuuint64_t strides[1] = {(cuuint64_t)kp * sizeof(float)};
+  const cuuint32_t box[2] = {(cuuint32_t)tc::BLOCK_K, 128u};
+  const cuuint32_t estr[2] = {1u, 1u};
+  CUresult r = reinterpret_cast<EncodeTiledFn>(ctx->tmap_encode)(
+      map, CU_TENSOR_MAP_DATA_TYPE_FLOAT16, 2, const_cast<float*>(plane), dims, strides, box, estr,
+      CU_TENSOR_MAP_INTERLEAVE_NONE, CU_TENSOR_MAP_SWIZZLE_64B, CU_TENSOR_MAP_L2_PROMOTION_L2_256B,
+      CU_TENSOR_MAP_FLOAT_OOB_FILL_NONE);
+  if (r != CUDA_SUCCESS) return fail(ctx, BOF_ECUDA, "cuTensorMapEncodeTiled failed with CUresult %d", (int)r);
+  return BOF_OK;
+}
+
+template <int CG, int EPI, bool CHUNKED, int SPLIT, bool FOLD = false>
 int launch_variant(bof_ctx* ctx, cudaStream_t s, const CUtensorMap* maps, const tc::Params& prm, int num_items) {
-  auto kern = tc::gemm3xtf32_kernel<CG, EPI, CHUNKED, HYB, FOLD>;
+  auto kern = tc::gemm3xtf32_kernel<CG, EPI, CHUNKED, SPLIT, FOLD>;
   static PerDeviceOnce attr_set;
   if (attr_set.need(ctx->device)) {
     BOF_CUDA(ctx, cudaFuncSetAttribute(kern, cudaFuncAttributeMaxDynamicSharedMemorySize, (int)tc::SMEM_BYTES));
@@ -779,18 +980,34 @@
                         int64_t s_r, int64_t s_k, float* hi, float* lo, int64_t kp) {
   BOF_REQUIRE(ctx, kp % 32 == 0 && kp >= K, "split: bad padded k");
   if (R == 0) return BOF_OK;
+  if (split_mode(ctx) == 3) {
+    const int64_t chunk = 32 * chunk_kb(kp, k_chunk_of(ctx)), n_chunks = ceil_div<int64_t>(kp, chunk);
+    if (s_k == 1) {
+      const int64_t warps = R * n_chunks;
+      const unsigned grid = (unsigned)std::min<int64_t>(ceil_div<int64_t>(warps, 8), (int64_t)ctx->num_sms * 32);
+      split3_kmajor_kernel<<<grid, 256, 0, s>>>(R, K, src, s_r, hi, lo, kp, chunk, n_chunks);
+      BOF_LAUNCH_CHECK(ctx, "split3_kmajor_kernel");
+    } else {
+      BOF_REQUIRE(ctx, s_r == 1, "split: one of the operand strides must be 1");
+      const int64_t blocks = ceil_div<int64_t>(R, 32) * n_chunks;
+      BOF_REQUIRE(ctx, blocks < (1ll << 31), "split: operand too large for one launch");
+      split3_transpose_kernel<<<(unsigned)blocks, 256, 0, s>>>(R, K, src, s_k, hi, lo, kp, chunk, n_chunks);
+      BOF_LAUNCH_CHECK(ctx, "split3_transpose_kernel");
+    }
+    return BOF_OK;
+  }
   if (s_k == 1) {
     const bool vec = (s_r % 4 == 0) && aligned16(src);
     const int64_t total = R * (kp / 4);
     const unsigned grid = (unsigned)std::min<int64_t>(ceil_div<int64_t>(total, 256), (int64_t)ctx->num_sms * 32);
-    split_planes_kmajor_kernel<<<grid, 256, 0, s>>>(R, K, src, s_r, hi, lo, kp, vec, hybrid_split(ctx));
+    split_planes_kmajor_kernel<<<grid, 256, 0, s>>>(R, K, src, s_r, hi, lo, kp, vec, split_mode(ctx) == 2);
     BOF_LAUNCH_CHECK(ctx, "split_planes_kmajor_kernel");
   } else {
     BOF_REQUIRE(ctx, s_r == 1, "split: one of the operand strides must be 1");
     const int64_t tiles_k = kp / 32, tiles_r = ceil_div<int64_t>(R, 32);
     BOF_REQUIRE(ctx, tiles_k * tiles_r < (1ll << 31), "split: operand too large for one launch");
     split_planes_transpose_kernel<<<(unsigned)(tiles_k * tiles_r), 256, 0, s>>>(R, K, src, s_k, hi, lo, kp,
-                                                                               (unsigned)tiles_k, hybrid_split(ctx));
+                                                                               (unsigned)tiles_k, split_mode(ctx) == 2);
     BOF_LAUNCH_CHECK(ctx, "split_planes_transpose_kernel");
   }
   return BOF_OK;
@@ -804,11 +1021,14 @@
   BOF_REQUIRE(ctx, cta_group == 1 || cta_group == 2, "gemm_tc: cta_group must be 1 or 2");
   BOF_REQUIRE(ctx, kp % 32 == 0 && kp > 0, "gemm_tc: padded k must be a positive multiple of 32");
   BOF_REQUIRE(ctx, M < (1ll << 31) && N < (1ll << 31) && kp < (1ll << 31), "gemm_tc: extent exceeds int32");
+  const int split = split_mode(ctx);
+  BOF_REQUIRE(ctx, split != 3 || chunk_kb(kp, k_chunk) == chunk_kb(kp, k_chunk_of(ctx)),
+              "gemm_tc: gemm_split = 3 needs the context's gemm_k_chunk");
   CUtensorMap maps[4];
   int rc;
-  if ((rc = make_plane_map(ctx, &maps[0], p_hi, M, kp))) return rc;
+  if ((rc = split == 3 ? make_hi16_map(ctx, &maps[0], p_hi, M, kp) : make_plane_map(ctx, &maps[0], p_hi, M, kp))) return rc;
   if ((rc = make_plane_map(ctx, &maps[1], p_lo, M, kp))) return rc;
-  if ((rc = make_plane_map(ctx, &maps[2], q_hi, N, kp))) return rc;
+  if ((rc = split == 3 ? make_hi16_map(ctx, &maps[2], q_hi, N, kp) : make_plane_map(ctx, &maps[2], q_hi, N, kp))) return rc;
   if ((rc = make_plane_map(ctx, &maps[3], q_lo, N, kp))) return rc;
 
   const int block_n = cta_group == 2 ? 256 : 128;
@@ -817,9 +1037,10 @@
   prm.M = M;
   prm.N = N;
   prm.num_kb = (int32_t)(kp / 32);
-  int64_t kbc = (k_chunk <= 0) ? prm.num_kb : std::max<int64_t>(1, k_chunk / 32);
-  if (kbc > prm.num_kb) kbc = prm.num_kb;
-  prm.kb_per_chunk = (int32_t)kbc;
+  prm.kb_per_chunk = (int32_t)chunk_kb(kp, k_chunk);
+  prm.p_exp = reinterpret_cast<const int16_t*>(p_hi) + kp;
+  prm.q_exp = reinterpret_cast<const int16_t*>(q_hi) + kp;
+  prm.exp_ld = 2 * kp;
   prm.tiles_m = (int32_t)ceil_div<int64_t>(M, tile_m);
   prm.tiles_n = (int32_t)ceil_div<int64_t>(N, block_n);
   const bool argmin = ep.C == nullptr;
@@ -860,19 +1081,21 @@
     prm.sync_counters = ctx->sync_ctr;
   }
 
-  const bool hyb = hybrid_split(ctx);
   if (fold) {
     if (cta_group == 2) {
-      if (hyb) return launch_variant<2, tc::EPI_GEMM, true, true, true>(ctx, s, maps, prm, num_items);
-      return launch_variant<2, tc::EPI_GEMM, true, false, true>(ctx, s, maps, prm, num_items);
-    }
-    if (hyb) return launch_variant<1, tc::EPI_GEMM, true, true, true>(ctx, s, maps, prm, num_items);
-    return launch_variant<1, tc::EPI_GEMM, true, false, true>(ctx, s, maps, prm, num_items);
-  }
-#define BOF_TC(CG, EPI, CH)                                                            \
-  do {                                                                                 \
-    if (hyb) return launch_variant<CG, EPI, CH, true>(ctx, s, maps, prm, num_items);   \
-    return launch_variant<CG, EPI, CH, false>(ctx, s, maps, prm, num_items);           \
+      if (split == 3) return launch_variant<2, tc::EPI_GEMM, true, 3, true>(ctx, s, maps, prm, num_items);
+      if (split == 2) return launch_variant<2, tc::EPI_GEMM, true, 2, true>(ctx, s, maps, prm, num_items);
+      return launch_variant<2, tc::EPI_GEMM, true, 1, true>(ctx, s, maps, prm, num_items);
+    }
+    if (split == 3) return launch_variant<1, tc::EPI_GEMM, true, 3, true>(ctx, s, maps, prm, num_items);
+    if (split == 2) return launch_variant<1, tc::EPI_GEMM, true, 2, true>(ctx, s, maps, prm, num_items);
+    return launch_variant<1, tc::EPI_GEMM, true, 1, true>(ctx, s, maps, prm, num_items);
+  }
+#define BOF_TC(CG, EPI, CH)                                                                  \
+  do {                                                                                       \
+    if (split == 3) return launch_variant<CG, EPI, CH, 3>(ctx, s, maps, prm, num_items);     \
+    if (split == 2) return launch_variant<CG, EPI, CH, 2>(ctx, s, maps, prm, num_items);     \
+    return launch_variant<CG, EPI, CH, 1>(ctx, s, maps, prm, num_items);                     \
   } while (0)
   if (cta_group == 2) {
     if (argmin) { if (chunked) BOF_TC(2, tc::EPI_ARGMIN, true); else BOF_TC(2, tc::EPI_ARGMIN, false); }
@@ -897,7 +1120,7 @@
 
 
 int tc_issue_rate(bof_ctx* ctx, cudaStream_t s, int kind, int rounds, double* mma_tflops, double* useful_tflops) {
-  BOF_REQUIRE(ctx, kind >= 0 && kind <= 2 && rounds > 0, "tc_issue_rate: bad kind / rounds");
+  BOF_REQUIRE(ctx, kind >= 0 && kind <= 3 && rounds > 0, "tc_issue_rate: bad kind / rounds");
   static PerDeviceOnce attr_set;
   const size_t smem = (size_t)tc::STAGE_BYTES + 2048;
   if (attr_set.need(ctx->device)) {
@@ -927,7 +1150,7 @@
   BOF_CUDA(ctx, cudaEventElapsedTime(&ms, e0, e1));
   cudaEventDestroy(e0); cudaEventDestroy(e1);
   const double per_round_useful = 2.0 * 256 * 256 * 32;
-  const double mma_per_round = per_round_useful * (kind == 2 ? 3.0 : (kind == 1 ? 2.0 : 1.0));
+  const double mma_per_round = per_round_useful * (kind >= 2 ? 3.0 : (kind == 1 ? 2.0 : 1.0));
   if (mma_tflops) *mma_tflops = mma_per_round * rounds * clusters / (ms * 1e-3) / 1e12;
   if (useful_tflops) *useful_tflops = per_round_useful * rounds * clusters / (ms * 1e-3) / 1e12;
   return BOF_OK;
diff --git a/blas-on-flash_b200/csrc/host_internal.cuh b/blas-on-flash_b200/csrc/host_internal.cuh
--- a/blas-on-flash_b200/csrc/host_internal.cuh
+++ b/blas-on-flash_b200/csrc/host_internal.cuh
@@ -71,7 +71,6 @@
 int64_t padded_k(int64_t k);
 size_t plane_bytes(int64_t rows, int64_t kp);
 int pick_gemm_path(const bof_ctx* ctx, int64_t Mo, int64_t No, int64_t K);
-int64_t k_chunk_of(const bof_ctx* ctx);
 int gemm_canon_device(bof_ctx* ctx, cudaStream_t s, const Canon& c, float alpha, float beta, float* C,
                       void* ws, size_t ws_bytes);
 
```

Result: slower. 339,600 (median of 6 runs) (-1.2%).
